# qiaozhijian/LPD-Net-Pytorch

Hardware: NVIDIA B200
Metric: LPD-Net eval embedding throughput (featnet=lpdnet, 4096 pts, k=20, NetVLAD K=64 D=1024 -> 256) (higher is better)
Workload: dtype f16

## Files before the change

### include/lpd_b200.h

```cpp
#ifndef LPD_B200_H
#define LPD_B200_H

#include <stddef.h>
#include <stdint.h>

#ifdef __cplusplus
extern "C" {
#endif

#define LPD_ABI_VERSION 2

typedef enum lpd_status {
    LPD_OK = 0,
    LPD_EINVAL = -1,
    LPD_EWORKSPACE = -2,
    LPD_ECUDA = -3,
    LPD_EUNSUPPORTED = -4
} lpd_status;

typedef enum lpd_act {
    LPD_ACT_NONE = 0,
    LPD_ACT_RELU = 1,
    LPD_ACT_LEAKY = 2,
    LPD_ACT_SIGMOID = 3,
    LPD_ACT_GATE = 4,
    LPD_ACT_ADD = 5
} lpd_act;

#define LPD_A_MK 0
#define LPD_A_KM 1
#define LPD_B_NK 0
#define LPD_B_KN 1

int lpd_abi_version(void);
const char* lpd_status_str(int status);
const char* lpd_last_cuda_error(void);
int lpd_device_info(int* sm_count, int* cc_major, int* cc_minor, size_t* smem_optin_bytes);

int lpd_bn_fold(const float* gamma, const float* beta, const float* mean, const float* var,
                const float* bias, float eps, int C, float* scale, float* shift, void* stream);

int lpd_transpose(const float* in, float* out, int batch, int rows, int cols, void* stream);

int lpd_knn(const float* x, int B, int N, int C, int k, void* idx, int idx_i64, void* stream);

size_t lpd_knn_workspace_bytes(int B, int N, int C, int k);
int lpd_knn_tc(const float* x, int B, int N, int C, int k, void* idx, int idx_i64,
               void* workspace, size_t workspace_bytes, void* stream);
int lpd_knn_tc_variant(int v);
size_t lpd_knn_tc_flags_offset(int B, int N, int C, int k);

size_t lpd_knn_xyz_workspace_bytes(int B, int N);
int lpd_knn_xyz(const float* x, int B, int N, int k, void* idx, int idx_i64, void* workspace, size_t workspace_bytes,
                void* stream);

int lpd_cell_order(const float* x, int B, int N, int32_t* perm, int32_t* inv, float* xyz_sorted,
                   void* workspace, size_t workspace_bytes, void* stream);

int lpd_cell_order_grid(const float* x, int B, int N, int32_t* perm, int32_t* inv, float* xyz_sorted,
                        void* workspace, size_t workspace_bytes, void* stream);
int lpd_knn_xyz_ordered(int B, int N, int k, void* idx, int idx_i64, void* workspace, size_t workspace_bytes, void* stream);

int lpd_gemm(const float* A, int a_layout, int lda, long long strideA,
             const float* B, int b_layout, int ldb, long long strideB,
             float* C, int ldc, long long strideC,
             int M, int N, int K, int batch,
             const float* scale, const float* shift, int act, float slope, const float* aux,
             void* stream);

int lpd_gemm_tf32(const float* A, int lda, const float* B, int ldb, float* C, int ldc,
                  int M, int N, int K, const float* scale, const float* shift, int act, float slope,
                  void* stream);
int lpd_gemm_tf32_ex(const float* A, int lda, const float* B, int ldb, float* C, int ldc,
                     int M, int N, int K, int batch, int accumulate, const float* scale, const float* shift, int act,
                     float slope, void* stream);

int lpd_gemm_tf32_tn(const float* A, int lda, const float* B, int ldb, float* C, int ldc, long long strideC,
                     int M, int N, int K, int batch, void* stream);

int lpd_gemm_f16(const void* A, int lda, const void* W, int ldw, void* C, int ldc, int out_half,
                 int M, int N, int K, const float* scale, const float* shift, int act, float slope, void* stream);
int lpd_gemm_f16_tn(const void* A, int lda, const void* B, int ldb, float* C, int ldc, long long strideC,
                    int M, int N, int K, int batch, void* stream);
int lpd_f32_to_f16(const float* x, long long ldx, void* y, long long ldy, long long rows, int cols, void* stream);
int lpd_split3_tf32(const float* x, long long n, float* out, int role, void* stream);
int lpd_transpose_split3(const float* v, int B, long long R, int Bp, float* out, void* stream);
int lpd_gemm_tf32_out16(const float* A, int lda, const float* B, int ldb, void* C, int ldc, int M, int N, int K,
                        const float* scale, const float* shift, int act, float slope, void* stream);
int lpd_softmax64_f16(float* a, long long M, void* a_h, void* stream);
int lpd_edge_gather_max_f16(const void* p, int ldp, const void* q, int ldq, const int32_t* idx, int B, int N, int k, int C,
                            int act, float slope, void* out, int ldo, void* stream);
int lpd_edgeconv_dg20_f16(const void* p, int ldp, const void* q, int ldq, const int32_t* idx, int B, int N,
                          const void* w2, const float* s2, const float* t2, int act, float slope,
                          void* x1, int ld1, void* x2, int ld2, void* stream);
int lpd_edgeconv_dg32_f16(const void* p, int ldp, const void* q, int ldq, const int32_t* idx, int B, int N,
                          const void* w2, const float* s2, const float* t2, int act, float slope,
                          void* x1, int ld1, void* x2, int ld2, void* stream);

int lpd_pointwise_mlp2(const float* x, int ldx, int D, long long M, const float* w1, const float* s1, const float* t1,
                       const float* w2, const float* s2, const float* t2, int act, float slope, float* out, int ldo,
                       void* stream);

int lpd_colmax(const float* x, int B, int N, int C, int ldx, float* out, void* stream);

int lpd_edge_gather_ext(const float* p, int ldp, const float* q, int ldq,
                        const int32_t* idx, int B, int N, int k, int C,
                        const float* scale, const float* shift, int act, float slope,
                        float* out, int ldo, void* stream);

int lpd_edgeconv_dg(const float* p, int ldp, const float* q, int ldq,
                    const int32_t* idx, int B, int N, int k, int C1, int C2,
                    const float* s1, const float* t1, const float* w2,
                    const float* s2, const float* t2, int act, float slope,
                    float* x1, int ld1, float* x2, int ld2, void* stream);

int lpd_edgeconv_dg_tf32(const float* p, int ldp, const float* q, int ldq,
                         const int32_t* idx, int B, int N, int k, int C1, int C2,
                         const float* s1, const float* t1, const float* w2,
                         const float* s2, const float* t2, int act, float slope,
                         float* x1, int ld1, float* x2, int ld2, void* stream);

int lpd_netvlad_assign(const float* x, int M, int D, const float* wc, const float* scale,
                       const float* shift, int K, float* a, void* stream);

int lpd_softmax64(float* a, long long M, void* stream);

int lpd_netvlad_finish(float* vlad, const float* a, const float* wc2, int B, int N, int D, int K,
                       float* asum_ws, void* stream);

int lpd_gemm_softmax64(const void* A, int a_f16, int lda, const void* W, int ldw, int M, int K, const float* scale,
                       const float* shift, float* a32, void* a16, float* apart, void* stream);

int lpd_netvlad_finish_parts(float* vlad, const float* apart, int nparts, const float* wc2, int B, int D, int K, void* stream);

int lpd_hidden_gate(const float* part, int splits, int B, int O, const float* s2, const float* t2, const float* wg,
                    const float* sg, const float* tg, float* out, void* stream);

int lpd_splitk_reduce(const float* part, int splits, int M, int N, const float* scale,
                      const float* shift, float* out, void* stream);

int lpd_quadruplet_loss(const float* q, const float* pos, const float* neg, const float* other,
                        int Bq, int P, int Nn, int D, float m1, float m2, int flags,
                        float* loss, float* gq, float* gpos, float* gneg, float* gother,
                        const float* grad_out, void* stream);

size_t lpd_retrieval_workspace_bytes(int Ndb, int Nq, int k);
int lpd_retrieval_topk(const float* db, int Ndb, const float* q, int Nq, int D, int k,
                       int idx_offset, int32_t* idx, double* dist,
                       void* workspace, size_t workspace_bytes, void* stream);

int lpd_topk_merge(const double* part_dist, const int32_t* part_idx, int lists, int Nq, int k,
                   int32_t* idx, double* dist, void* stream);

size_t lpd_retrieval_tc_workspace_bytes(int Ndb, int Nq, int D);
int lpd_retrieval_tc(const float* db, int Ndb, const float* q, int Nq, int D, int k,
                     const int32_t* seg_off, int S, int global_idx, int idx_offset,
                     int32_t* idx, double* dist, void* workspace, size_t workspace_bytes, void* stream);

int lpd_recall_count(const int32_t* idx, int S, int Nq, int k, const int32_t* q_run, int R, const int32_t* seg_run,
                     const int32_t* truth_off, const int32_t* truth_idx, const int32_t* seg_thresh,
                     const float* db, const int32_t* seg_off, const float* q, int D,
                     int32_t* hist, int32_t* n_eval, int32_t* n_onepct, float* sim, void* stream);


int lpd_bn_stats(const float* z, long long rows, int C, int ld, double* partial, int nparts, void* stream);
int lpd_bn_finalize(const double* partial, int nparts, double count, int C, const float* gamma, const float* beta,
                    float eps, float momentum, float* running_mean, float* running_var, float* bn_out, void* stream);
int lpd_colsum_finalize(const double* partial, int nparts, int n, float* out, void* stream);
int lpd_affine_act(const float* z, long long rows, int C, int ldz, const float* scale, const float* shift, int act,
                   float slope, const float* aux, int ldaux, float* out, int ldo, void* stream);
int lpd_bn_bwd_reduce(const float* dy, int lddy, const float* z, int ldz, long long rows, int C, const float* bn,
                      int act, float slope, const float* aux, int ldaux, double* partial, int nparts, void* stream);
int lpd_bn_bwd_apply(const float* dy, int lddy, const float* z, int ldz, long long rows, int C, const float* bn,
                     const float* S, double count, int act, float slope, const float* aux, int ldaux,
                     float* dz, int lddz, void* stream);

int lpd_edge_sel_stats(const float* p, int ldp, const float* q, int ldq, const int32_t* idx, int B, int N, int k, int C,
                       const float* gamma, float* zsel, int ldz, uint8_t* arg, double* partial, int nparts, void* stream);
int lpd_edge_materialize(const float* p, int ldp, const float* q, int ldq, const int32_t* idx, int B, int N, int k, int C,
                         const float* scale, const float* shift, int act, float slope, float* y, void* stream);
int lpd_edge_sel_dense(const float* z, long long M, int k, int C, const float* gamma, float* zsel, int ldz,
                       uint8_t* arg, void* stream);
int lpd_edge_dense_bwd_apply(const float* z, long long M, int k, int C, const float* bn, const float* S, double count,
                             int act, float slope, const float* dx, int lddx, const float* zsel, int ldzs,
                             const uint8_t* arg, float* dz, void* stream);
int lpd_edge_bwd_reduce(const float* p, int ldp, const float* q, int ldq, const int32_t* idx, int B, int N, int k, int C,
                        const float* bn, int act, float slope, const float* dx, int lddx, const uint8_t* arg,
                        const float* dy, double* partial, int nparts, void* stream);
int lpd_edge_bwd_apply(const float* p, int ldp, const float* q, int ldq, const int32_t* idx, int B, int N, int k, int C,
                       const float* bn, int act, float slope, const float* dx, int lddx, const uint8_t* arg,
                       const float* dy, const float* S, double count, float* dp, int lddp, float* dq, int lddq,
                       void* stream);

int lpd_edge_scatter_add(const float* dy, const int32_t* idx, int B, int N, int k, int C, float* dp, int lddp, void* stream);

int lpd_netvlad_finish_train(float* vlad, const float* a, const float* wc2, int B, int N, int D, int K,
                             float* asum, float* n1, float* n2, void* stream);
int lpd_netvlad_finish_bwd(float* dv, const float* v, const float* wc2, const float* asum, const float* n1,
                           const float* n2, int B, int D, int K, float* dasum, float* dwc2, void* stream);
int lpd_softmax64_bwd(float* da, const float* a, const float* dasum, long long M, int N, void* stream);

int lpd_colmax_arg(const float* x, int B, int N, int C, int ldx, float* out, int32_t* arg, void* stream);
int lpd_colmax_bwd(const float* dout, const int32_t* arg, int B, int N, int C, float* dx, int lddx, void* stream);

int lpd_adam(float* w, const float* g, float* m, float* v, long long n, float lr, float beta1, float beta2, float eps,
             float weight_decay, int step, float grad_scale, void* stream);
int lpd_axpy(float* y, int ldy, const float* x, int ldx, long long rows, int C, float alpha, void* stream);

#ifdef __cplusplus
}
#endif
#endif
```

### lpd-net-pytorch_b200/_lib.py

```python
from __future__ import annotations

import ctypes as C
import os
from pathlib import Path

_HERE = Path(__file__).resolve().parent
LIB_PATH = _HERE / "liblpd_b200.so"

LPD_OK = 0
ACT_NONE, ACT_RELU, ACT_LEAKY, ACT_SIGMOID, ACT_GATE, ACT_ADD = 0, 1, 2, 3, 4, 5
A_MK, A_KM = 0, 1
B_NK, B_KN = 0, 1
ABI_VERSION = 2

_vp, _i, _f, _ll, _sz, _d = C.c_void_p, C.c_int, C.c_float, C.c_longlong, C.c_size_t, C.c_double

SIGNATURES = {
    "lpd_abi_version": (_i, []),
    "lpd_status_str": (C.c_char_p, [_i]),
    "lpd_last_cuda_error": (C.c_char_p, []),
    "lpd_device_info": (_i, [C.POINTER(_i), C.POINTER(_i), C.POINTER(_i), C.POINTER(_sz)]),
    "lpd_bn_fold": (_i, [_vp, _vp, _vp, _vp, _vp, _f, _i, _vp, _vp, _vp]),
    "lpd_transpose": (_i, [_vp, _vp, _i, _i, _i, _vp]),
    "lpd_knn": (_i, [_vp, _i, _i, _i, _i, _vp, _i, _vp]),
    "lpd_knn_workspace_bytes": (_sz, [_i, _i, _i, _i]),
    "lpd_knn_tc": (_i, [_vp, _i, _i, _i, _i, _vp, _i, _vp, _sz, _vp]),
    "lpd_knn_tc_variant": (_i, [_i]),
    "lpd_knn_tc_flags_offset": (_sz, [_i, _i, _i, _i]),
    "lpd_knn_xyz_workspace_bytes": (_sz, [_i, _i]),
    "lpd_knn_xyz": (_i, [_vp, _i, _i, _i, _vp, _i, _vp, _sz, _vp]),
    "lpd_cell_order": (_i, [_vp, _i, _i, _vp, _vp, _vp, _vp, _sz, _vp]),
    "lpd_cell_order_grid": (_i, [_vp, _i, _i, _vp, _vp, _vp, _vp, _sz, _vp]),
    "lpd_knn_xyz_ordered": (_i, [_i, _i, _i, _vp, _i, _vp, _sz, _vp]),
    "lpd_gemm": (_i, [_vp, _i, _i, _ll, _vp, _i, _i, _ll, _vp, _i, _ll, _i, _i, _i, _i,
                      _vp, _vp, _i, _f, _vp, _vp]),
    "lpd_gemm_tf32": (_i, [_vp, _i, _vp, _i, _vp, _i, _i, _i, _i, _vp, _vp, _i, _f, _vp]),
    "lpd_gemm_tf32_ex": (_i, [_vp, _i, _vp, _i, _vp, _i, _i, _i, _i, _i, _i, _vp, _vp, _i, _f, _vp]),
    "lpd_gemm_tf32_tn": (_i, [_vp, _i, _vp, _i, _vp, _i, _ll, _i, _i, _i, _i, _vp]),
    "lpd_gemm_f16": (_i, [_vp, _i, _vp, _i, _vp, _i, _i, _i, _i, _i, _vp, _vp, _i, _f, _vp]),
    "lpd_gemm_f16_tn": (_i, [_vp, _i, _vp, _i, _vp, _i, _ll, _i, _i, _i, _i, _vp]),
    "lpd_f32_to_f16": (_i, [_vp, _ll, _vp, _ll, _ll, _i, _vp]),
    "lpd_split3_tf32": (_i, [_vp, _ll, _vp, _i, _vp]),
    "lpd_transpose_split3": (_i, [_vp, _i, _ll, _i, _vp, _vp]),
    "lpd_gemm_tf32_out16": (_i, [_vp, _i, _vp, _i, _vp, _i, _i, _i, _i, _vp, _vp, _i, _f, _vp]),
    "lpd_softmax64_f16": (_i, [_vp, _ll, _vp, _vp]),
    "lpd_edge_gather_max_f16": (_i, [_vp, _i, _vp, _i, _vp, _i, _i, _i, _i, _i, _f, _vp, _i, _vp]),
    "lpd_edgeconv_dg20_f16": (_i, [_vp, _i, _vp, _i, _vp, _i, _i, _vp, _vp, _vp, _i, _f, _vp, _i, _vp, _i, _vp]),
    "lpd_edgeconv_dg32_f16": (_i, [_vp, _i, _vp, _i, _vp, _i, _i, _vp, _vp, _vp, _i, _f, _vp, _i, _vp, _i, _vp]),
    "lpd_pointwise_mlp2": (_i, [_vp, _i, _i, _ll, _vp, _vp, _vp, _vp, _vp, _vp, _i, _f, _vp, _i, _vp]),
    "lpd_colmax": (_i, [_vp, _i, _i, _i, _i, _vp, _vp]),
    "lpd_edge_gather_ext": (_i, [_vp, _i, _vp, _i, _vp, _i, _i, _i, _i, _vp, _vp, _i, _f, _vp, _i, _vp]),
    "lpd_edgeconv_dg": (_i, [_vp, _i, _vp, _i, _vp, _i, _i, _i, _i, _i, _vp, _vp, _vp, _vp, _vp, _i, _f,
                             _vp, _i, _vp, _i, _vp]),
    "lpd_edgeconv_dg_tf32": (_i, [_vp, _i, _vp, _i, _vp, _i, _i, _i, _i, _i, _vp, _vp, _vp, _vp, _vp, _i, _f,
                                  _vp, _i, _vp, _i, _vp]),
    "lpd_netvlad_assign": (_i, [_vp, _i, _i, _vp, _vp, _vp, _i, _vp, _vp]),
    "lpd_softmax64": (_i, [_vp, _ll, _vp]),
    "lpd_netvlad_finish": (_i, [_vp, _vp, _vp, _i, _i, _i, _i, _vp, _vp]),
    "lpd_splitk_reduce": (_i, [_vp, _i, _i, _i, _vp, _vp, _vp, _vp]),
    "lpd_gemm_softmax64": (_i, [_vp, _i, _i, _vp, _i, _i, _i, _vp, _vp, _vp, _vp, _vp, _vp]),
    "lpd_netvlad_finish_parts": (_i, [_vp, _vp, _i, _vp, _i, _i, _i, _vp]),
    "lpd_hidden_gate": (_i, [_vp, _i, _i, _i, _vp, _vp, _vp, _vp, _vp, _vp, _vp]),
    "lpd_quadruplet_loss": (_i, [_vp, _vp, _vp, _vp, _i, _i, _i, _i, _f, _f, _i, _vp, _vp, _vp, _vp, _vp, _vp, _vp]),
    "lpd_retrieval_workspace_bytes": (_sz, [_i, _i, _i]),
    "lpd_retrieval_topk": (_i, [_vp, _i, _vp, _i, _i, _i, _i, _vp, _vp, _vp, _sz, _vp]),
    "lpd_topk_merge": (_i, [_vp, _vp, _i, _i, _i, _vp, _vp, _vp]),
    "lpd_retrieval_tc_workspace_bytes": (_sz, [_i, _i, _i]),
    "lpd_retrieval_tc": (_i, [_vp, _i, _vp, _i, _i, _i, _vp, _i, _i, _i, _vp, _vp, _vp, _sz, _vp]),
    "lpd_recall_count": (_i, [_vp, _i, _i, _i, _vp, _i, _vp, _vp, _vp, _vp, _vp, _vp, _vp, _i, _vp, _vp, _vp, _vp, _vp]),
    "lpd_bn_stats": (_i, [_vp, _ll, _i, _i, _vp, _i, _vp]),
    "lpd_bn_finalize": (_i, [_vp, _i, _d, _i, _vp, _vp, _f, _f, _vp, _vp, _vp, _vp]),
    "lpd_colsum_finalize": (_i, [_vp, _i, _i, _vp, _vp]),
    "lpd_affine_act": (_i, [_vp, _ll, _i, _i, _vp, _vp, _i, _f, _vp, _i, _vp, _i, _vp]),
    "lpd_bn_bwd_reduce": (_i, [_vp, _i, _vp, _i, _ll, _i, _vp, _i, _f, _vp, _i, _vp, _i, _vp]),
    "lpd_bn_bwd_apply": (_i, [_vp, _i, _vp, _i, _ll, _i, _vp, _vp, _d, _i, _f, _vp, _i, _vp, _i, _vp]),
    "lpd_edge_sel_stats": (_i, [_vp, _i, _vp, _i, _vp, _i, _i, _i, _i, _vp, _vp, _i, _vp, _vp, _i, _vp]),
    "lpd_edge_materialize": (_i, [_vp, _i, _vp, _i, _vp, _i, _i, _i, _i, _vp, _vp, _i, _f, _vp, _vp]),
    "lpd_edge_sel_dense": (_i, [_vp, _ll, _i, _i, _vp, _vp, _i, _vp, _vp]),
    "lpd_edge_dense_bwd_apply": (_i, [_vp, _ll, _i, _i, _vp, _vp, _d, _i, _f, _vp, _i, _vp, _i, _vp, _vp, _vp]),
    "lpd_edge_bwd_reduce": (_i, [_vp, _i, _vp, _i, _vp, _i, _i, _i, _i, _vp, _i, _f, _vp, _i, _vp, _vp, _vp, _i, _vp]),
    "lpd_edge_bwd_apply": (_i, [_vp, _i, _vp, _i, _vp, _i, _i, _i, _i, _vp, _i, _f, _vp, _i, _vp, _vp, _vp, _d,
                                _vp, _i, _vp, _i, _vp]),
    "lpd_edge_scatter_add": (_i, [_vp, _vp, _i, _i, _i, _i, _vp, _i, _vp]),
    "lpd_netvlad_finish_train": (_i, [_vp, _vp, _vp, _i, _i, _i, _i, _vp, _vp, _vp, _vp]),
    "lpd_netvlad_finish_bwd": (_i, [_vp, _vp, _vp, _vp, _vp, _vp, _i, _i, _i, _vp, _vp, _vp]),
    "lpd_softmax64_bwd": (_i, [_vp, _vp, _vp, _ll, _i, _vp]),
    "lpd_colmax_arg": (_i, [_vp, _i, _i, _i, _i, _vp, _vp, _vp]),
    "lpd_colmax_bwd": (_i, [_vp, _vp, _i, _i, _i, _vp, _i, _vp]),
    "lpd_adam": (_i, [_vp, _vp, _vp, _vp, _ll, _f, _f, _f, _f, _f, _i, _f, _vp]),
    "lpd_axpy": (_i, [_vp, _i, _vp, _i, _ll, _i, _f, _vp]),
}

_lib = None


class LpdError(RuntimeError):
    pass


def load() -> C.CDLL:
    global _lib
    if _lib is not None:
        return _lib
    path = Path(os.environ.get("LPD_B200_LIB", LIB_PATH))
    if not path.exists():
        raise LpdError(
            f"{path} not found: build it with `python -c 'import __graft_entry__ as g; g.build()'` "
            f"or `make -C {_HERE / 'csrc'}`; there is no CPU or torch fallback.")
    lib = C.CDLL(str(path))
    for name, (res, args) in SIGNATURES.items():
        fn = getattr(lib, name)
        fn.restype = res
        fn.argtypes = args
    if lib.lpd_abi_version() != ABI_VERSION:
        raise LpdError(f"ABI version mismatch: library {lib.lpd_abi_version()} != binding {ABI_VERSION}")
    _lib = lib
    return lib


def check(rc: int, what: str) -> None:
    if rc != LPD_OK:
        lib = load()
        msg = lib.lpd_status_str(rc).decode()
        detail = lib.lpd_last_cuda_error().decode()
        raise LpdError(f"{what} failed: {msg}" + (f" [{detail}]" if detail else ""))


def device_info() -> dict:
    lib = load()
    sm, maj, mnr, smem = _i(), _i(), _i(), _sz()
    check(lib.lpd_device_info(C.byref(sm), C.byref(maj), C.byref(mnr), C.byref(smem)), "lpd_device_info")
    return {"sm_count": sm.value, "cc": (maj.value, mnr.value), "smem_optin": smem.value}
```

### lpd-net-pytorch_b200/csrc/knn_tc.cu

```cuda
#include "tc_common.cuh"
#include "knn_select.cuh"

namespace lpd {

int knn_simt64_flagged(const float* x, int B, int N, int k, void* idx, int idx_i64, const int* flags, cudaStream_t st);

namespace tc {

constexpr int KT_Q = 128;
constexpr int KT_C = 64;
constexpr int KT_SCAN_WARPS = 8;
constexpr int KT_THREADS = 320;
constexpr int KT_STRIDE = 257;
constexpr int KT_BSTAGES = 3;
constexpr int KT_TSTAGES = 4;
constexpr int KT_XSLOTS = 8;

struct KnnTcParams {
    const float* xxpad;
    float* cand_v;
    int* cand_i;
    int B, N, Npad;
    int qtiles, ctiles;
};

__device__ __forceinline__ int ct_of(int s, int center, int ctiles) {
    const int d = (s + 1) >> 1;
    int ct = center + ((s & 1) ? d : -d);
    ct %= ctiles;
    return ct < 0 ? ct + ctiles : ct;
}

__device__ __forceinline__ float to_tf32(float v) {
    uint32_t r;
    asm("cvt.rna.tf32.f32 %0, %1;" : "=r"(r) : "f"(v));
    return __uint_as_float(r);
}

__global__ void __launch_bounds__(256)
knn_split_kernel(const float* __restrict__ x, int N, int Npad, float* __restrict__ x2, float* __restrict__ xxpad,
                 float* __restrict__ r2) {
    const int b = blockIdx.y;
    const int n = blockIdx.x * blockDim.x + threadIdx.x;
    if (n >= Npad) return;
    float v = INFINITY;
    if (n < N) {
        const float4* p = reinterpret_cast<const float4*>(x + ((size_t)b * N + n) * 64);
        float4* o = reinterpret_cast<float4*>(x2 + ((size_t)b * N + n) * 128);
        float acc = 0.f;
#pragma unroll
        for (int g = 0; g < 16; ++g) {
            const float4 t = __ldg(p + g);
            acc = __fmaf_rn(t.x, t.x, acc); acc = __fmaf_rn(t.y, t.y, acc);
            acc = __fmaf_rn(t.z, t.z, acc); acc = __fmaf_rn(t.w, t.w, acc);
            float4 hi, lo;
            hi.x = to_tf32(t.x); hi.y = to_tf32(t.y); hi.z = to_tf32(t.z); hi.w = to_tf32(t.w);
            lo.x = to_tf32(t.x - hi.x); lo.y = to_tf32(t.y - hi.y); lo.z = to_tf32(t.z - hi.z); lo.w = to_tf32(t.w - hi.w);
            o[g] = hi;
            o[16 + g] = lo;
        }
        v = acc;
        atomicMax(reinterpret_cast<int*>(r2 + b), __float_as_int(acc));
    }
    xxpad[(size_t)b * Npad + n] = v;
}

template <int GS, int QD>
struct KtSmem {
    static constexpr int L = 4 * GS;
    static constexpr uint32_t A_KB = KT_Q * 128;
    static constexpr uint32_t B_KB = KT_C * 128;
    static constexpr uint32_t A_BYTES = 4 * A_KB;
    static constexpr uint32_t B_BYTES = 4 * B_KB;
    static constexpr size_t off_b = A_BYTES;
    static constexpr size_t off_xs = off_b + KT_BSTAGES * B_BYTES;
    static constexpr size_t off_lv = off_xs + KT_XSLOTS * KT_C * 4;
    static constexpr size_t off_li = off_lv + (size_t)L * KT_STRIDE * 4;
    static constexpr size_t off_bar = (off_li + (size_t)L * KT_STRIDE * 4 + 7) / 8 * 8;
    static constexpr size_t total = off_bar + (2 + 2 * KT_BSTAGES + 2 * KT_TSTAGES) * 8 + 16;
    static_assert(total <= 227 * 1024, "knn_tc shared memory budget");
};

template <int GS, int QD>
__global__ void __launch_bounds__(KT_THREADS, 1)
knn_tc_kernel(const __grid_constant__ CUtensorMap tmap_a, const __grid_constant__ CUtensorMap tmap_b, KnnTcParams P) {
    using S = KtSmem<GS, QD>;
    constexpr int L = S::L;
    extern __shared__ __align__(1024) uint8_t smem[];
    if ((smem_u32(smem) & 1023u) != 0) __trap();
    uint8_t* a_s = smem;
    uint8_t* b_s = smem + S::off_b;
    float* xs = reinterpret_cast<float*>(smem + S::off_xs);
    float* lv = reinterpret_cast<float*>(smem + S::off_lv);
    int* li = reinterpret_cast<int*>(smem + S::off_li);
    uint64_t* afull = reinterpret_cast<uint64_t*>(smem + S::off_bar);
    uint64_t* aempty = afull + 1;
    uint64_t* bfull = aempty + 1;
    uint64_t* bempty = bfull + KT_BSTAGES;
    uint64_t* tfull = bempty + KT_BSTAGES;
    uint64_t* tempty = tfull + KT_TSTAGES;
    uint32_t* tmem_slot = reinterpret_cast<uint32_t*>(tempty + KT_TSTAGES);

    const int warp = threadIdx.x >> 5, lane = threadIdx.x & 31;
    const int items = P.B * P.qtiles;

    if (warp == 9) {
        if (lane == 0) {
            asm volatile("prefetch.tensormap [%0];" ::"l"(reinterpret_cast<uint64_t>(&tmap_a)) : "memory");
            asm volatile("prefetch.tensormap [%0];" ::"l"(reinterpret_cast<uint64_t>(&tmap_b)) : "memory");
            mbar_init(afull, 1); mbar_init(aempty, 1);
            for (int s = 0; s < KT_BSTAGES; ++s) { mbar_init(&bfull[s], 1); mbar_init(&bempty[s], 1); }
            for (int s = 0; s < KT_TSTAGES; ++s) { mbar_init(&tfull[s], 1); mbar_init(&tempty[s], KT_SCAN_WARPS); }
            asm volatile("fence.mbarrier_init.release.cluster;" ::: "memory");
        }
        __syncwarp();
        asm volatile("tcgen05.alloc.cta_group::1.sync.aligned.shared::cta.b32 [%0], 256;" ::"r"(smem_u32(tmem_slot)) : "memory");
        asm volatile("tcgen05.relinquish_alloc_permit.cta_group::1.sync.aligned;" ::: "memory");
    }
    tc_fence_before();
    __syncthreads();
    tc_fence_after();
    const uint32_t tmem_base = *tmem_slot;

    if (warp == 8) {
        if (lane == 0) {
            uint32_t tcount = 0, icount = 0;
            for (int item = blockIdx.x; item < items; item += gridDim.x, ++icount) {
                const int b = item / P.qtiles, q0 = (item % P.qtiles) * KT_Q;
                mbar_wait_sleep(aempty, (icount & 1) ^ 1);
                mbar_expect_tx(afull, S::A_BYTES);
#pragma unroll
                for (int kb = 0; kb < 4; ++kb) tma_load_2d(a_s + kb * S::A_KB, &tmap_a, afull, kb * 32, b * P.N + q0);
                for (int cs = 0; cs < P.ctiles; ++cs, ++tcount) {
                    const int ct = ct_of(cs, q0 / KT_C, P.ctiles);
                    const uint32_t s = tcount % KT_BSTAGES, ph = (tcount / KT_BSTAGES) & 1;
                    mbar_wait_sleep(&bempty[s], ph ^ 1);
                    mbar_expect_tx(&bfull[s], S::B_BYTES + KT_C * 4);
                    uint8_t* bs = b_s + s * S::B_BYTES;
#pragma unroll
                    for (int kb = 0; kb < 4; ++kb) tma_load_2d(bs + kb * S::B_KB, &tmap_b, &bfull[s], kb * 32, b * P.N + ct * KT_C);
                    asm volatile("cp.async.bulk.shared::cluster.global.mbarrier::complete_tx::bytes [%0], [%1], %2, [%3];"
                                 ::"r"(smem_u32(xs + (tcount % KT_XSLOTS) * KT_C)), "l"(P.xxpad + (size_t)b * P.Npad + ct * KT_C),
                                   "r"(KT_C * 4), "r"(smem_u32(&bfull[s])) : "memory");
                }
            }
        }
    } else if (warp == 9) {
        if (lane == 0) {
            constexpr uint32_t idesc = make_idesc(KT_Q, KT_C);
            const uint32_t a_addr = smem_u32(a_s);
            uint32_t tcount = 0, icount = 0;
            for (int item = blockIdx.x; item < items; item += gridDim.x, ++icount) {
                mbar_wait_sleep(afull, icount & 1);
                for (int ct = 0; ct < P.ctiles; ++ct, ++tcount) {
                    const uint32_t s = tcount % KT_BSTAGES, ph = (tcount / KT_BSTAGES) & 1;
                    const uint32_t ts = tcount % KT_TSTAGES, tph = (tcount / KT_TSTAGES) & 1;
                    mbar_wait_sleep(&tempty[ts], tph ^ 1);
                    mbar_wait_sleep(&bfull[s], ph);
                    tc_fence_after();
                    const uint32_t b_addr = smem_u32(b_s + s * S::B_BYTES);
                    const uint32_t d = tmem_base + ts * KT_C;
                    uint32_t acc = 0;
#pragma unroll
                    for (int term = 0; term < 3; ++term) {
                        const int akb = (term == 1) ? 2 : 0, bkb = (term == 0) ? 2 : 0;
#pragma unroll
                        for (int kb = 0; kb < 2; ++kb) {
                            const uint64_t da = make_smem_desc(a_addr + (akb + kb) * S::A_KB);
                            const uint64_t db = make_smem_desc(b_addr + (bkb + kb) * S::B_KB);
#pragma unroll
                            for (int ks = 0; ks < 4; ++ks) {
                                tc_mma_tf32(d, da + (uint64_t)(ks * 2), db + (uint64_t)(ks * 2), idesc, acc);
                                acc = 1;
                            }
                        }
                    }
                    tc_commit(&bempty[s]);
                    tc_commit(&tfull[ts]);
                }
                tc_commit(aempty);
            }
        }
    } else {
        const int quad = warp & 3, half = warp >> 2;
        const int own = half * KT_Q + quad * 32 + lane;
        RowSelect<GS, false, KT_STRIDE> sel;
        uint32_t tcount = 0;
        for (int item = blockIdx.x; item < items; item += gridDim.x) {
            const int b = item / P.qtiles, q0 = (item % P.qtiles) * KT_Q;
            sel.reset();
            for (int cs = 0; cs < P.ctiles; ++cs, ++tcount) {
                const int ct = ct_of(cs, q0 / KT_C, P.ctiles);
                const uint32_t ts = tcount % KT_TSTAGES, tph = (tcount / KT_TSTAGES) & 1;
                mbar_wait(&tfull[ts], tph);
                tc_fence_after();
                const float* xsj = xs + (tcount % KT_XSLOTS) * KT_C + half * 32;
                uint32_t r[32];
                tc_ld32(tmem_base + ((uint32_t)(quad * 32) << 16) + ts * KT_C + half * 32, r);
                tc_fence_before();
                __syncwarp();
                if (lane == 0) mbar_arrive(&tempty[ts]);
                const int jbase = ct * KT_C + half * 32;
#pragma unroll
                for (int sub = 0; sub < 32 / QD; ++sub) {
                    float a[QD];
                    float m4[4] = {-INFINITY, -INFINITY, -INFINITY, -INFINITY};
#pragma unroll
                    for (int j = 0; j < QD; j += 4) {
                        const float4 xx = *reinterpret_cast<const float4*>(xsj + sub * QD + j);
                        a[j + 0] = fmaf(2.f, __uint_as_float(r[sub * QD + j + 0]), -xx.x);
                        a[j + 1] = fmaf(2.f, __uint_as_float(r[sub * QD + j + 1]), -xx.y);
                        a[j + 2] = fmaf(2.f, __uint_as_float(r[sub * QD + j + 2]), -xx.z);
                        a[j + 3] = fmaf(2.f, __uint_as_float(r[sub * QD + j + 3]), -xx.w);
                        m4[0] = fmaxf(m4[0], a[j]); m4[1] = fmaxf(m4[1], a[j + 1]);
                        m4[2] = fmaxf(m4[2], a[j + 2]); m4[3] = fmaxf(m4[3], a[j + 3]);
                    }
                    const float mx = fmaxf(fmaxf(m4[0], m4[1]), fmaxf(m4[2], m4[3]));
                    uint32_t mask = 0;
                    if (mx > sel.tau) {
#pragma unroll
                        for (int j = 0; j < QD; ++j) mask |= (a[j] > sel.tau) ? (1u << j) : 0u;
                    }
                    while (__any_sync(kFull, mask != 0)) {
                        if (mask) {
                            const int j = __ffs(mask) - 1;
                            mask &= mask - 1;
                            float t[QD];
#pragma unroll
                            for (int q = 0; q < QD; ++q) t[q] = a[q];
#pragma unroll
                            for (int w = QD / 2, bit = 0; w >= 1; w >>= 1, ++bit) {
                                const bool hi = (j >> bit) & 1;
#pragma unroll
                                for (int q = 0; q < w; ++q) t[q] = hi ? t[2 * q + 1] : t[2 * q];
                            }
                            sel.insert(lv, li, own, t[0], jbase + sub * QD + j);
                        }
                    }
                }
            }
            __syncwarp();
            for (int rl = 0; rl < 32; ++rl) {
                const int qrow = q0 + quad * 32 + rl;
                const int nfill = __shfl_sync(kFull, sel.filled, rl);
                if (qrow >= P.N) break;
                const size_t o = (((size_t)b * P.N + qrow) * 2 + half) * L;
                const int src = half * KT_Q + quad * 32 + rl;
                for (int s = lane; s < L; s += 32) {
                    const bool valid = s < nfill;
                    P.cand_v[o + s] = valid ? lv[s * KT_STRIDE + src] : -INFINITY;
                    P.cand_i[o + s] = valid ? li[s * KT_STRIDE + src] : INT_MAX;
                }
            }
            __syncwarp();
        }
    }
    tc_fence_before();
    __syncthreads();
    if (warp == 9) {
        tc_fence_after();
        asm volatile("tcgen05.dealloc.cta_group::1.sync.aligned.b32 %0, 256;" ::"r"(tmem_base) : "memory");
    }
}

__global__ void __launch_bounds__(256)
knn_refine_kernel(const float* __restrict__ x, const float* __restrict__ xxpad, const float* __restrict__ r2,
                  const float* __restrict__ cand_v, const int* __restrict__ cand_i, int Lh, int B, int N, int Npad, int k,
                  void* __restrict__ idx_out, int idx_i64, int* __restrict__ flags) {
    constexpr int E = 2;
    const int lane = threadIdx.x & 31;
    const long long grow = (long long)blockIdx.x * 8 + (threadIdx.x >> 5);
    if (grow >= (long long)B * N) return;
    const int b = (int)(grow / N), qi = (int)(grow % N);
    const int L = 2 * Lh;
    float av[E]; int id[E];
    float tmin[2] = {INFINITY, INFINITY};
    bool hfull[2] = {true, true};
#pragma unroll
    for (int e = 0; e < E; ++e) {
        const int s = e * 32 + lane;
        av[e] = -INFINITY; id[e] = INT_MAX;
        if (s < L) {
            av[e] = cand_v[grow * L + s];
            id[e] = cand_i[grow * L + s];
            const int h = s >= Lh;
            if (id[e] == INT_MAX || id[e] >= N) {
                id[e] = INT_MAX;
                if (h) hfull[1] = false; else hfull[0] = false;
            } else {
                if (h) tmin[1] = fminf(tmin[1], av[e]); else tmin[0] = fminf(tmin[0], av[e]);
            }
        }
    }
#pragma unroll
    for (int o = 16; o > 0; o >>= 1) {
        tmin[0] = fminf(tmin[0], __shfl_xor_sync(kFull, tmin[0], o));
        tmin[1] = fminf(tmin[1], __shfl_xor_sync(kFull, tmin[1], o));
    }
    const bool full0 = __all_sync(kFull, hfull[0]), full1 = __all_sync(kFull, hfull[1]);
    const float tau = fmaxf(full0 ? tmin[0] : -INFINITY, full1 ? tmin[1] : -INFINITY);
    const float xxi = __ldg(xxpad + (size_t)b * Npad + qi);
    const float rmax2 = __ldg(r2 + b);
    const float eps = 6.103515625e-5f * sqrtf(xxi) * sqrtf(rmax2) + 9.5367431640625e-7f * (xxi + rmax2);
    warp_sort_desc<E>(av, id, lane);
    const float a_k = __shfl_sync(kFull, av[0], k - 1);
    const float cut = a_k - 2.f * eps;
    const float4* xi = reinterpret_cast<const float4*>(x + ((size_t)b * N + qi) * 64);
    float pd[E];
#pragma unroll
    for (int e = 0; e < E; ++e) {
        pd[e] = -INFINITY;
        const bool keep = (id[e] != INT_MAX) && (av[e] >= cut);
        if (!keep) id[e] = INT_MAX;
        if (__any_sync(kFull, keep)) {
            if (keep) {
                const float4* xj = reinterpret_cast<const float4*>(x + ((size_t)b * N + id[e]) * 64);
                float dot = 0.f;
#pragma unroll
                for (int g = 0; g < 16; ++g) {
                    const float4 u = __ldg(xi + g), w = __ldg(xj + g);
                    dot = __fmaf_rn(u.x, w.x, dot); dot = __fmaf_rn(u.y, w.y, dot);
                    dot = __fmaf_rn(u.z, w.z, dot); dot = __fmaf_rn(u.w, w.w, dot);
                }
                const float xxj = __ldg(xxpad + (size_t)b * Npad + id[e]);
                const float t = -2.0f * dot;
                pd[e] = __fsub_rn(__fsub_rn(-xxj, t), xxi);
            }
        }
    }
    warp_sort_desc<E>(pd, id, lane);
    const float pd_k = __shfl_sync(kFull, pd[0], k - 1);
    const bool ok = (tau == -INFINITY) || (tau + eps < pd_k + xxi);
    const size_t o = (size_t)grow * k;
#pragma unroll
    for (int e = 0; e < E; ++e) {
        const int g = e * 32 + lane;
        if (g < k) {
            if (idx_i64) reinterpret_cast<long long*>(idx_out)[o + g] = id[e];
            else reinterpret_cast<int*>(idx_out)[o + g] = id[e];
        }
    }
    if (!ok && lane == 0) flags[(size_t)b * ((N + 63) / 64) + qi / 64] = 1;
}

template <int GS, int QD>
static int knn_tc_launch(const CUtensorMap& ta, const CUtensorMap& tb, const KnnTcParams& P, cudaStream_t st) {
    const size_t smem = KtSmem<GS, QD>::total;
    LPD_CUDA_CHECK(allow_smem(knn_tc_kernel<GS, QD>, smem));
    int dev = 0, sms = 0;
    LPD_CUDA_CHECK(cudaGetDevice(&dev));
    LPD_CUDA_CHECK(cudaDeviceGetAttribute(&sms, cudaDevAttrMultiProcessorCount, dev));
    const int items = P.B * P.qtiles;
    knn_tc_kernel<GS, QD><<<items < sms ? items : sms, KT_THREADS, smem, st>>>(ta, tb, P);
    LPD_LAUNCH_CHECK();
    return LPD_OK;
}

static inline size_t align_up(size_t v, size_t a) { return (v + a - 1) / a * a; }

struct KnnWs {
    size_t off_xx, off_r2, off_flags, off_x2, off_cv, off_ci, total;
    int npad, L;
    KnnWs(int B, int N, int k) {
        npad = (N + 127) / 128 * 128;
        L = k <= 24 ? 48 : 64;
        size_t o = 0;
        off_xx = o; o = align_up(o + (size_t)B * npad * 4, 256);
        off_r2 = o; o += (size_t)B * 4;
        off_flags = o; o = align_up(o + (size_t)B * ((N + 63) / 64) * 4, 256);
        off_x2 = o; o = align_up(o + (size_t)B * N * 128 * 4, 256);
        off_cv = o; o = align_up(o + (size_t)B * N * L * 4, 256);
        off_ci = o; o = align_up(o + (size_t)B * N * L * 4, 256);
        total = o;
    }
};

}
}

namespace lpd { namespace tc {
size_t knn2_workspace_bytes(int B, int N, int k);
size_t knn2_flags_offset(int B, int N, int k);
int knn2_run(const float* x, int B, int N, int k, void* idx, int idx_i64, void* workspace, size_t workspace_bytes, int mt,
             cudaStream_t st);
static int g_knn_variant = 1;
}}

extern "C" int lpd_knn_tc_variant(int v) {
    const int prev = lpd::tc::g_knn_variant;
    if (v >= 0 && v <= 3) lpd::tc::g_knn_variant = v;
    return prev;
}

extern "C" size_t lpd_knn_workspace_bytes(int B, int N, int C, int k) {
    if (B < 1 || N < 1 || C != 64 || k < 1 || k > 32) return 0;
    const size_t a = lpd::tc::KnnWs(B, N, k).total, b = lpd::tc::knn2_workspace_bytes(B, N, k);
    return a > b ? a : b;
}

extern "C" size_t lpd_knn_tc_flags_offset(int B, int N, int C, int k) {
    if (B < 1 || N < 1 || C != 64 || k < 1 || k > 32) return 0;
    return lpd::tc::g_knn_variant == 0 ? lpd::tc::KnnWs(B, N, k).off_flags : lpd::tc::knn2_flags_offset(B, N, k);
}

extern "C" int lpd_knn_tc(const float* x, int B, int N, int C, int k, void* idx, int idx_i64,
                          void* workspace, size_t workspace_bytes, void* stream) {
    using namespace lpd;
    LPD_REQUIRE(x && idx && workspace);
    LPD_REQUIRE(B >= 1 && B <= 65535 && N >= 1 && C == 64 && k >= 1 && k <= 32 && k <= N);
    LPD_REQUIRE((long long)B * N < (1ll << 31) / 128);
    LPD_REQUIRE(((uintptr_t)x & 15) == 0 && ((uintptr_t)workspace & 255) == 0);
    const tc::KnnWs W(B, N, k);
    if (workspace_bytes < lpd_knn_workspace_bytes(B, N, C, k)) return LPD_EWORKSPACE;
    int dev = 0, major = 0;
    LPD_CUDA_CHECK(cudaGetDevice(&dev));
    LPD_CUDA_CHECK(cudaDeviceGetAttribute(&major, cudaDevAttrComputeCapabilityMajor, dev));
    if (major != 10) return LPD_EUNSUPPORTED;
    cudaStream_t st = as_stream(stream);
    if (tc::g_knn_variant != 0) return tc::knn2_run(x, B, N, k, idx, idx_i64, workspace, workspace_bytes, tc::g_knn_variant, st);
    uint8_t* ws = reinterpret_cast<uint8_t*>(workspace);
    float* xxpad = reinterpret_cast<float*>(ws + W.off_xx);
    float* r2 = reinterpret_cast<float*>(ws + W.off_r2);
    int* flags = reinterpret_cast<int*>(ws + W.off_flags);
    float* x2 = reinterpret_cast<float*>(ws + W.off_x2);
    const int ftiles = (N + 63) / 64;
    LPD_CUDA_CHECK(cudaMemsetAsync(r2, 0, (size_t)B * sizeof(float), st));
    LPD_CUDA_CHECK(cudaMemsetAsync(flags, 0, (size_t)B * ftiles * sizeof(int), st));
    tc::knn_split_kernel<<<dim3(ceil_div(W.npad, 256), B), 256, 0, st>>>(x, N, W.npad, x2, xxpad, r2);
    LPD_LAUNCH_CHECK();
    CUtensorMap ta, tb;
    int rc = tc::make_tmap(&ta, x2, (long long)B * N, 128, 128, tc::KT_Q);
    if (rc != LPD_OK) return rc;
    rc = tc::make_tmap(&tb, x2, (long long)B * N, 128, 128, tc::KT_C);
    if (rc != LPD_OK) return rc;
    tc::KnnTcParams P;
    P.xxpad = xxpad;
    P.cand_v = reinterpret_cast<float*>(ws + W.off_cv);
    P.cand_i = reinterpret_cast<int*>(ws + W.off_ci);
    P.B = B; P.N = N; P.Npad = W.npad; P.qtiles = ceil_div(N, tc::KT_Q); P.ctiles = ceil_div(N, tc::KT_C);
    rc = (W.L == 48) ? tc::knn_tc_launch<6, 16>(ta, tb, P, st) : tc::knn_tc_launch<8, 16>(ta, tb, P, st);
    if (rc != LPD_OK) return rc;
    const unsigned rblocks = (unsigned)(((long long)B * N + 7) / 8);
    tc::knn_refine_kernel<<<rblocks, 256, 0, st>>>(x, xxpad, r2, P.cand_v, P.cand_i, W.L / 2, B, N, W.npad, k, idx, idx_i64, flags);
    LPD_LAUNCH_CHECK();
    return knn_simt64_flagged(x, B, N, k, idx, idx_i64, flags, st);
}
```

### lpd-net-pytorch_b200/csrc/knn_tc2.cu

```cuda
#include "tc_common.cuh"
#include <cuda_fp16.h>
#include <limits.h>
#include <stdlib.h>

namespace lpd {

int knn_simt64_list(const float* x, int B, int N, int k, void* idx, int idx_i64, const int* list, cudaStream_t st);

namespace tc {

constexpr int K2_C = 128;
constexpr int K2_BSTAGES = 4;
constexpr int K2_TCOLS = 512;
constexpr int K2_XSLOTS = 12;
constexpr int K2_TBL = 128;

struct Knn2Params {
    const float* nrmpad;
    const float* snpad;
    const uint4* xh;
    const uint4* ext;
    const float* xxpad;
    const float* r2;
    const float* r2c;
    const float* sc;
    int* cnt;
    int* cand;
    int B, N, Npad, k;
    int qtiles, ctiles;
};

__device__ __forceinline__ void tc_mma_f16(uint32_t tmem_d, uint64_t desc_a, uint64_t desc_b, uint32_t idesc, uint32_t accumulate) {
    asm volatile(
        "{\n\t.reg .pred p;\n\t"
        "setp.ne.b32 p, %4, 0;\n\t"
        "tcgen05.mma.cta_group::1.kind::f16 [%0], %1, %2, %3, p;\n\t}"
        ::"r"(tmem_d), "l"(desc_a), "l"(desc_b), "r"(idesc), "r"(accumulate)
        : "memory");
}
__device__ __forceinline__ void tc_mma_f16_p(uint32_t tmem_d, uint64_t desc_a, uint64_t desc_b, uint32_t idesc, uint32_t accumulate,
                                             uint32_t leader) {
    asm volatile(
        "{\n\t.reg .pred p, q;\n\t"
        "setp.ne.b32 p, %4, 0;\n\t"
        "elect.sync _|q, 0xffffffff;\n\t"
        "@q tcgen05.mma.cta_group::1.kind::f16 [%0], %1, %2, %3, p;\n\t}"
        ::"r"(tmem_d), "l"(desc_a), "l"(desc_b), "r"(idesc), "r"(accumulate), "r"(leader)
        : "memory");
}
__device__ __forceinline__ void tc_commit_p(uint64_t* bar, uint32_t leader) {
    asm volatile(
        "{\n\t.reg .pred q;\n\t"
        "elect.sync _|q, 0xffffffff;\n\t"
        "@q tcgen05.commit.cta_group::1.mbarrier::arrive::one.shared::cluster.b64 [%0];\n\t}"
        ::"r"(smem_u32(bar)), "r"(leader) : "memory");
}
__device__ __forceinline__ void tma_load_2d_p(void* smem_dst, const CUtensorMap* tmap, uint64_t* bar, int c0, int c1, uint32_t leader) {
    asm volatile(
        "{\n\t.reg .pred q;\n\t"
        "elect.sync _|q, 0xffffffff;\n\t"
        "@q cp.async.bulk.tensor.2d.shared::cluster.global.mbarrier::complete_tx::bytes [%0], [%1, {%3, %4}], [%2];\n\t}"
        ::"r"(smem_u32(smem_dst)), "l"(reinterpret_cast<uint64_t>(tmap)), "r"(smem_u32(bar)), "r"(c0), "r"(c1), "r"(leader)
        : "memory");
}
__device__ __forceinline__ void bulk_load_p(void* smem_dst, const void* gsrc, uint32_t bytes, uint64_t* bar, uint32_t leader) {
    asm volatile(
        "{\n\t.reg .pred q;\n\t"
        "elect.sync _|q, 0xffffffff;\n\t"
        "@q cp.async.bulk.shared::cluster.global.mbarrier::complete_tx::bytes [%0], [%1], %2, [%3];\n\t}"
        ::"r"(smem_u32(smem_dst)), "l"(gsrc), "r"(bytes), "r"(smem_u32(bar)), "r"(leader) : "memory");
}
__device__ __forceinline__ void mbar_expect_tx_p(uint64_t* bar, uint32_t bytes, uint32_t leader) {
    asm volatile(
        "{\n\t.reg .pred q;\n\t"
        "elect.sync _|q, 0xffffffff;\n\t"
        "@q mbarrier.arrive.expect_tx.shared::cta.b64 _, [%0], %1;\n\t}"
        ::"r"(smem_u32(bar)), "r"(bytes), "r"(leader) : "memory");
}
__device__ __forceinline__ void tc_mma_f16_ts(uint32_t tmem_d, uint32_t tmem_a, uint64_t desc_b, uint32_t idesc, uint32_t accumulate) {
    asm volatile(
        "{\n\t.reg .pred p, q;\n\t"
        "setp.ne.b32 p, %4, 0;\n\t"
        "elect.sync _|q, 0xffffffff;\n\t"
        "@q tcgen05.mma.cta_group::1.kind::f16 [%0], [%1], %2, %3, p;\n\t}"
        ::"r"(tmem_d), "r"(tmem_a), "l"(desc_b), "r"(idesc), "r"(accumulate)
        : "memory");
}
__device__ __forceinline__ void tc_st4(uint32_t taddr, const uint4& v) {
    asm volatile("tcgen05.st.sync.aligned.32x32b.x4.b32 [%0], {%1, %2, %3, %4};"
                 ::"r"(taddr), "r"(v.x), "r"(v.y), "r"(v.z), "r"(v.w) : "memory");
}
__host__ __device__ constexpr uint32_t make_idesc_f16(int M, int N) {
    return (1u << 4) | ((uint32_t)(N >> 3) << 17) | ((uint32_t)(M >> 4) << 24);
}
__device__ __forceinline__ void named_bar(int id, int nthreads) {
    asm volatile("bar.sync %0, %1;" ::"r"(id), "r"(nthreads) : "memory");
}

__host__ __device__ __forceinline__ void block_perm(int t, int& a, int& b) {
    const uint32_t v = (uint32_t)(t + 1) * 2654435761u;
    a = (int)((v >> 8) & 63u) | 1;
    b = (int)((v >> 20) & 63u);
}
__host__ __device__ __forceinline__ int inv_mod64(int a) {
    return (a * (2 - a * a)) & 63;
}

constexpr int K2_CSPLIT = 8;
__global__ void __launch_bounds__(256)
knn2_center_kernel(const float* __restrict__ x, int N, float* __restrict__ part) {
    __shared__ float4 red[3][256];
    __shared__ int sbad;
    const int b = blockIdx.y, sp = blockIdx.x, t = threadIdx.x, cg = t & 15, rl = t >> 4;
    const int chunk = (N + K2_CSPLIT - 1) / K2_CSPLIT;
    const int n0 = sp * chunk, n1 = min(N, n0 + chunk);
    const float4* xb = reinterpret_cast<const float4*>(x + (size_t)b * N * 64);
    if (t == 0) sbad = 0;
    float4 s = make_float4(0.f, 0.f, 0.f, 0.f);
    float4 lo = make_float4(INFINITY, INFINITY, INFINITY, INFINITY), hi = make_float4(-INFINITY, -INFINITY, -INFINITY, -INFINITY);
    bool bad = false;
    for (int n = n0 + rl; n < n1; n += 16) {
        const float4 v = __ldg(xb + (size_t)n * 16 + cg);
        s.x += v.x; s.y += v.y; s.z += v.z; s.w += v.w;
        lo.x = fminf(lo.x, v.x); lo.y = fminf(lo.y, v.y); lo.z = fminf(lo.z, v.z); lo.w = fminf(lo.w, v.w);
        hi.x = fmaxf(hi.x, v.x); hi.y = fmaxf(hi.y, v.y); hi.z = fmaxf(hi.z, v.z); hi.w = fmaxf(hi.w, v.w);
        bad |= !(fabsf(v.x) <= 3.0e38f) || !(fabsf(v.y) <= 3.0e38f) || !(fabsf(v.z) <= 3.0e38f) || !(fabsf(v.w) <= 3.0e38f);
    }
    red[0][t] = s; red[1][t] = lo; red[2][t] = hi;
    __syncthreads();
    if (bad) sbad = 1;
    for (int o = 128; o >= 16; o >>= 1) {
        if (t < o) {
            const float4 a0 = red[0][t], c0 = red[0][t + o], a1 = red[1][t], c1 = red[1][t + o], a2 = red[2][t], c2 = red[2][t + o];
            red[0][t] = make_float4(a0.x + c0.x, a0.y + c0.y, a0.z + c0.z, a0.w + c0.w);
            red[1][t] = make_float4(fminf(a1.x, c1.x), fminf(a1.y, c1.y), fminf(a1.z, c1.z), fminf(a1.w, c1.w));
            red[2][t] = make_float4(fmaxf(a2.x, c2.x), fmaxf(a2.y, c2.y), fmaxf(a2.z, c2.z), fmaxf(a2.w, c2.w));
        }
        __syncthreads();
    }
    float* o = part + ((size_t)b * K2_CSPLIT + sp) * 196;
    if (t < 16) {
        reinterpret_cast<float4*>(o)[t] = red[0][t];
        reinterpret_cast<float4*>(o + 64)[t] = red[1][t];
        reinterpret_cast<float4*>(o + 128)[t] = red[2][t];
    }
    if (t == 0) o[192] = sbad ? 1.f : 0.f;
}

__device__ __forceinline__ void knn2_fold_center(const float* __restrict__ part, int b, int N, float* mus, float* ssc, float* red) {
    const int t = threadIdx.x;
    if (t < 64) {
        const float* pb = part + (size_t)b * K2_CSPLIT * 196;
        float s = 0.f, lo = INFINITY, hi = -INFINITY, bad = 0.f;
#pragma unroll
        for (int sp = 0; sp < K2_CSPLIT; ++sp) {
            s += pb[sp * 196 + t];
            lo = fminf(lo, pb[sp * 196 + 64 + t]);
            hi = fmaxf(hi, pb[sp * 196 + 128 + t]);
            bad += pb[sp * 196 + 192];
        }
        const float m = s * (1.f / (float)N);
        mus[t] = m;
        float g = fmaxf(hi - m, m - lo);
        if (bad != 0.f || !(g <= 3.0e38f)) g = INFINITY;
        red[t] = g;
    }
    __syncthreads();
    if (t == 0) {
        float g = 0.f;
        for (int c = 0; c < 64; ++c) g = fmaxf(g, red[c]);
        float sigma = 1.f, c2 = 2.f;
        if (g > 0.f) {
            int e;
            frexpf(g, &e);
            const int se = 8 - e;
            if (!(g <= 3.0e38f) || se > 60 || se < -60) {
                sigma = 1.f; c2 = __int_as_float(0x7fc00000);
            } else {
                sigma = ldexpf(1.f, se);
                c2 = ldexpf(2.f, -2 * se);
            }
        }
        ssc[0] = sigma; ssc[1] = c2;
    }
    __syncthreads();
}

constexpr int K2_PREP_XS = 68;
constexpr int K2_PREP_HS = 9;
constexpr size_t K2_PREP_SMEM = 256 * K2_PREP_XS * 4 + 256 * K2_PREP_HS * 16;
__global__ void __launch_bounds__(256)
knn2_prep_kernel(const float* __restrict__ x, const float* __restrict__ part, float* __restrict__ sc, int N, int Npad,
                 __half* __restrict__ xh, uint4* __restrict__ ext, float* __restrict__ xxpad, float* __restrict__ nrmpad,
                 float* __restrict__ snpad, float* __restrict__ r2, float* __restrict__ r2c) {
    __shared__ __align__(16) float mus_f[64];
    __shared__ float ssc[2], sred[64];
    extern __shared__ __align__(16) uint8_t prep_sm[];
    float* xs = reinterpret_cast<float*>(prep_sm);
    uint4* hs = reinterpret_cast<uint4*>(prep_sm + 256 * K2_PREP_XS * 4);
    const int b = blockIdx.y;
    const int n0 = blockIdx.x * 256;
    {
        const float4* src = reinterpret_cast<const float4*>(x + ((size_t)b * N + n0) * 64);
        const int rows = min(256, N - n0);
#pragma unroll 4
        for (int i = threadIdx.x; i < rows * 16; i += 256)
            *reinterpret_cast<float4*>(xs + (i >> 4) * K2_PREP_XS + (i & 15) * 4) = __ldg(src + i);
    }
    knn2_fold_center(part, b, N, mus_f, ssc, sred);
    const float4* mus = reinterpret_cast<const float4*>(mus_f);
    const float sigma = ssc[0];
    if (blockIdx.x == 0 && threadIdx.x == 0) { sc[2 * b] = sigma; sc[2 * b + 1] = ssc[1]; }
    const int n = n0 + threadIdx.x;
    float vxx = INFINITY, vn = INFINITY;
    int np = n;
    if ((n | 63) < N) {
        int a, bb;
        block_perm(n >> 6, a, bb);
        np = (n & ~63) | (((n & 63) * a + bb) & 63);
    }
    if (n < N) {
        const float4* p = reinterpret_cast<const float4*>(xs + threadIdx.x * K2_PREP_XS);
        uint4* o = hs + (np - n0) * K2_PREP_HS;
        float acc = 0.f, accc = 0.f;
#pragma unroll
        for (int g = 0; g < 8; ++g) {
            const float4 t0 = p[2 * g], t1 = p[2 * g + 1];
            acc = __fmaf_rn(t0.x, t0.x, acc); acc = __fmaf_rn(t0.y, t0.y, acc);
            acc = __fmaf_rn(t0.z, t0.z, acc); acc = __fmaf_rn(t0.w, t0.w, acc);
            acc = __fmaf_rn(t1.x, t1.x, acc); acc = __fmaf_rn(t1.y, t1.y, acc);
            acc = __fmaf_rn(t1.z, t1.z, acc); acc = __fmaf_rn(t1.w, t1.w, acc);
            const float4 m0 = mus[2 * g], m1 = mus[2 * g + 1];
            float c[8] = {t0.x - m0.x, t0.y - m0.y, t0.z - m0.z, t0.w - m0.w, t1.x - m1.x, t1.y - m1.y, t1.z - m1.z, t1.w - m1.w};
#pragma unroll
            for (int q = 0; q < 8; ++q) accc = __fmaf_rn(c[q], c[q], accc);
            uint32_t pk[4];
#pragma unroll
            for (int q = 0; q < 4; ++q) {
                const __half2 h = __floats2half2_rn(c[2 * q] * sigma, c[2 * q + 1] * sigma);
                pk[q] = *reinterpret_cast<const uint32_t*>(&h);
            }
            o[g] = make_uint4(pk[0], pk[1], pk[2], pk[3]);
        }
        vxx = acc; vn = accc;
        atomicMax(reinterpret_cast<int*>(r2 + b), __float_as_int(acc));
        atomicMax(reinterpret_cast<int*>(r2c + b), __float_as_int(accc));
    }
    __syncthreads();
    {
        uint4* dst = reinterpret_cast<uint4*>(xh + ((size_t)b * N + n0) * 64);
        const int rows = min(256, N - n0);
#pragma unroll 4
        for (int i = threadIdx.x; i < rows * 8; i += 256) dst[i] = hs[(i >> 3) * K2_PREP_HS + (i & 7)];
    }
    {
        float b1 = 0.f, b2 = 0.f, b3 = 0.f, b4 = -60000.f;
        if (n < N) {
            const float V = 0.5f * (sigma * sigma) * vn;
            b1 = __half2float(__float2half_rn(V * 0.015625f));
            const float r1 = __fmaf_rn(-b1, 64.f, V);
            b2 = __half2float(__float2half_rn(r1 * 32.f));
            const float rr = __fmaf_rn(-b2, 0.03125f, r1);
            b3 = __half2float(__float2half_rn(rr * 16384.f));
            b4 = 0.f;
        }
        const __half2 h01 = __floats2half2_rn(-b1, -b2), h23 = __floats2half2_rn(-b3, b4);
        const int r = np & 63;
        uint4* e = ext + ((size_t)b * (Npad >> 6) + (np >> 6)) * 128 + (r >> 3) * 16 + (r & 7);
        e[0] = make_uint4(*reinterpret_cast<const uint32_t*>(&h01), *reinterpret_cast<const uint32_t*>(&h23), 0u, 0u);
        e[8] = make_uint4(0u, 0u, 0u, 0u);
    }
    xxpad[(size_t)b * Npad + n] = vxx;
    nrmpad[(size_t)b * Npad + np] = vn;
    snpad[(size_t)b * Npad + np] = n < N ? sqrtf(vn) : 0.f;
}

__device__ __forceinline__ void cex_desc(float& a, float& b) {
    const float hi = fmaxf(a, b), lo = fminf(a, b);
    a = hi; b = lo;
}
__device__ __forceinline__ void bitonic_merge32_desc(float (&v)[32]) {
#pragma unroll
    for (int stride = 16; stride > 0; stride >>= 1) {
#pragma unroll
        for (int i = 0; i < 32; ++i)
            if ((i & stride) == 0) cex_desc(v[i], v[i | stride]);
    }
}
__device__ __forceinline__ void bitonic_sort32_desc(float (&v)[32]) {
#pragma unroll
    for (int size = 2; size <= 32; size <<= 1) {
#pragma unroll
        for (int stride = size >> 1; stride > 0; stride >>= 1) {
#pragma unroll
            for (int i = 0; i < 32; ++i) {
                if ((i & stride) == 0) {
                    const bool desc = ((i & size) == 0) || (size == 32);
                    if (desc) cex_desc(v[i], v[i | stride]); else cex_desc(v[i | stride], v[i]);
                }
            }
        }
    }
}

__device__ __forceinline__ uint64_t make_smem_desc_ext(uint32_t smem_addr) {
    uint64_t d = 0;
    d |= (uint64_t)((smem_addr & 0x3FFFF) >> 4);
    d |= (uint64_t)(128 >> 4) << 16;
    d |= (uint64_t)(256 >> 4) << 32;
    d |= (uint64_t)1 << 46;
    return d;
}
__device__ __forceinline__ void tc_ld32x2(uint32_t taddr, uint32_t (&a)[32], uint32_t (&b)[32]) {
#define LPD_LD32(R, ADDR)                                                                                               \
    asm volatile(                                                                                                       \
        "tcgen05.ld.sync.aligned.32x32b.x32.b32 "                                                                       \
        "{%0, %1, %2, %3, %4, %5, %6, %7, %8, %9, %10, %11, %12, %13, %14, %15, "                                       \
        "%16, %17, %18, %19, %20, %21, %22, %23, %24, %25, %26, %27, %28, %29, %30, %31}, [%32];"                       \
        : "=r"(R[0]), "=r"(R[1]), "=r"(R[2]), "=r"(R[3]), "=r"(R[4]), "=r"(R[5]), "=r"(R[6]), "=r"(R[7]),              \
          "=r"(R[8]), "=r"(R[9]), "=r"(R[10]), "=r"(R[11]), "=r"(R[12]), "=r"(R[13]), "=r"(R[14]), "=r"(R[15]),        \
          "=r"(R[16]), "=r"(R[17]), "=r"(R[18]), "=r"(R[19]), "=r"(R[20]), "=r"(R[21]), "=r"(R[22]), "=r"(R[23]),      \
          "=r"(R[24]), "=r"(R[25]), "=r"(R[26]), "=r"(R[27]), "=r"(R[28]), "=r"(R[29]), "=r"(R[30]), "=r"(R[31])       \
        : "r"(ADDR))
    LPD_LD32(a, taddr);
    LPD_LD32(b, taddr + 64);
#undef LPD_LD32
    asm volatile("tcgen05.wait::ld.sync.aligned;" ::: "memory");
}
__device__ __forceinline__ int fkey(float v) {
    const int b = __float_as_int(v);
    return b ^ ((b >> 31) & 0x7fffffff);
}
__device__ __forceinline__ float fmax3(float a, float b, float c) {
    float r;
    asm("max.f32 %0, %1, %2, %3;" : "=f"(r) : "f"(a), "f"(b), "f"(c));
    return r;
}

template <int MT, bool TS = false>
struct K2Smem {
    static constexpr int SCAN_THREADS = 256 * MT;
    static constexpr int TSTAGES = TS ? 3 : K2_TCOLS / (K2_C * MT);
    static constexpr int EXS = SCAN_THREADS + 1;
    static constexpr uint32_t A_TILE = 128 * 128;
    static constexpr uint32_t A_BYTES = MT * A_TILE;
    static constexpr uint32_t B_BYTES = K2_C * 128;
    static constexpr uint32_t BX_BYTES = K2_C * 32;
    static constexpr size_t off_b = TS ? 0 : 2 * A_BYTES;
    static constexpr size_t off_bx = off_b + K2_BSTAGES * B_BYTES;
    static constexpr size_t off_ax = off_bx + K2_BSTAGES * BX_BYTES;
    static constexpr size_t off_xs = off_ax + 128 * 32;
    static constexpr size_t off_ex = off_xs + K2_XSLOTS * K2_C * 4;
    static constexpr size_t off_tbl = off_ex + (size_t)32 * EXS * 4;
    static constexpr size_t off_bar = (off_tbl + (size_t)8 * MT * K2_TBL * 4 + 7) / 8 * 8;
    static constexpr size_t total = off_bar + (4 + 2 * K2_BSTAGES + 2 * TSTAGES) * 8 + 16;
    static_assert(total <= 227 * 1024, "knn2 shared memory budget");
};

template <int MT, int CAP, bool TIGHT, bool TS>
__global__ void __launch_bounds__(256 * MT + 64, 1)
knn2_tc_kernel(const __grid_constant__ CUtensorMap tmap_a, const __grid_constant__ CUtensorMap tmap_b, Knn2Params P) {
    static_assert(!TS || MT == 1, "TS mode: one 128-row query tile per item");
    using S = K2Smem<MT, TS>;
    constexpr int SCAN_WARPS = 8 * MT;
    constexpr uint32_t ACOL = 384;
    constexpr int TCOLS = K2_C * MT;
    constexpr int K2_TSTAGES = S::TSTAGES;
    extern __shared__ __align__(1024) uint8_t smem[];
    if ((smem_u32(smem) & 1023u) != 0) __trap();
    uint8_t* a_s = smem;
    uint8_t* b_s = smem + S::off_b;
    uint8_t* bx_s = smem + S::off_bx;
    uint8_t* ax_s = smem + S::off_ax;
    float* xs = reinterpret_cast<float*>(smem + S::off_xs);
    float* ex = reinterpret_cast<float*>(smem + S::off_ex);
    int* tbl = reinterpret_cast<int*>(smem + S::off_tbl);
    uint64_t* afull = reinterpret_cast<uint64_t*>(smem + S::off_bar);
    uint64_t* aempty = afull + 2;
    uint64_t* bfull = aempty + 2;
    uint64_t* bempty = bfull + K2_BSTAGES;
    uint64_t* tfull = bempty + K2_BSTAGES;
    uint64_t* tempty = tfull + K2_TSTAGES;
    uint32_t* tmem_slot = reinterpret_cast<uint32_t*>(tempty + K2_TSTAGES);

    const int warp = threadIdx.x >> 5, lane = threadIdx.x & 31;
    const int items = P.B * P.qtiles;
    const int nstages = 2 * P.ctiles;
    const int full_blocks = P.N >> 6;

    if (threadIdx.x < 128) {
        const int r = threadIdx.x;
        const __half2 h01 = __floats2half2_rn(64.f, 0.03125f), h23 = __floats2half2_rn(6.103515625e-05f, 32768.f);
        uint4* e = reinterpret_cast<uint4*>(ax_s) + (r >> 3) * 16 + (r & 7);
        e[0] = make_uint4(*reinterpret_cast<const uint32_t*>(&h01), *reinterpret_cast<const uint32_t*>(&h23), 0u, 0u);
        e[8] = make_uint4(0u, 0u, 0u, 0u);
        asm volatile("fence.proxy.async.shared::cta;" ::: "memory");
    }
    if (warp == SCAN_WARPS + 1) {
        if (lane == 0) {
            asm volatile("prefetch.tensormap [%0];" ::"l"(reinterpret_cast<uint64_t>(&tmap_a)) : "memory");
            asm volatile("prefetch.tensormap [%0];" ::"l"(reinterpret_cast<uint64_t>(&tmap_b)) : "memory");
            for (int s = 0; s < 2; ++s) { mbar_init(&afull[s], TS ? SCAN_WARPS : 1); mbar_init(&aempty[s], 1); }
            for (int s = 0; s < K2_BSTAGES; ++s) { mbar_init(&bfull[s], 1); mbar_init(&bempty[s], 1); }
            for (int s = 0; s < K2_TSTAGES; ++s) { mbar_init(&tfull[s], 1); mbar_init(&tempty[s], SCAN_WARPS); }
            asm volatile("fence.mbarrier_init.release.cluster;" ::: "memory");
        }
        __syncwarp();
        asm volatile("tcgen05.alloc.cta_group::1.sync.aligned.shared::cta.b32 [%0], %1;" ::"r"(smem_u32(tmem_slot)), "r"(TS ? 512 : TCOLS * K2_TSTAGES) : "memory");
        asm volatile("tcgen05.relinquish_alloc_permit.cta_group::1.sync.aligned;" ::: "memory");
    }
    tc_fence_before();
    __syncthreads();
    tc_fence_after();
    const uint32_t tmem_base = *tmem_slot;

    if (warp == SCAN_WARPS) {
        {
            const uint32_t leader = lane == 0;
            uint32_t tcount = 0, icount = 0;
            for (int item = blockIdx.x; item < items; item += gridDim.x, ++icount) {
                const int b = item / P.qtiles, q0 = (item % P.qtiles) * (128 * MT);
                const uint32_t ab = icount & 1, aph = (icount >> 1) & 1;
                if (!TS) {
                    mbar_wait_sleep(&aempty[ab], aph ^ 1);
                    mbar_expect_tx_p(&afull[ab], S::A_BYTES, leader);
#pragma unroll
                    for (int mt = 0; mt < MT; ++mt)
                        tma_load_2d_p(a_s + ab * S::A_BYTES + mt * S::A_TILE, &tmap_a, &afull[ab], 0, b * P.N + q0 + mt * 128, leader);
                }
                const uint4* extb = P.ext + (size_t)b * (P.Npad >> 6) * 128;
                const float* snb = P.snpad + (size_t)b * P.Npad;
                uint32_t s = tcount % K2_BSTAGES, ph = (tcount / K2_BSTAGES) & 1, xsl = tcount % K2_XSLOTS;
                for (int cs = 0; cs < nstages; ++cs, ++tcount) {
                    const int ct = cs >= P.ctiles ? cs - P.ctiles : cs;
                    mbar_wait_sleep(&bempty[s], ph ^ 1);
                    mbar_expect_tx_p(&bfull[s], S::B_BYTES + S::BX_BYTES + (TIGHT ? K2_C * 4 : 0), leader);
                    tma_load_2d_p(b_s + s * S::B_BYTES, &tmap_b, &bfull[s], 0, b * P.N + ct * K2_C, leader);
                    bulk_load_p(bx_s + s * S::BX_BYTES, extb + (size_t)ct * 256, S::BX_BYTES, &bfull[s], leader);
                    if (TIGHT) bulk_load_p(xs + xsl * K2_C, snb + ct * K2_C, K2_C * 4, &bfull[s], leader);
                    if (++s == K2_BSTAGES) { s = 0; ph ^= 1; }
                    xsl = (xsl + 1) % K2_XSLOTS;
                }
            }
        }
    } else if (warp == SCAN_WARPS + 1) {
        {
            constexpr uint32_t idesc = make_idesc_f16(128, K2_C);
            const uint32_t leader = lane == 0;
            const uint64_t dax = make_smem_desc_ext(smem_u32(ax_s));
            uint32_t tcount = 0, icount = 0;
            for (int item = blockIdx.x; item < items; item += gridDim.x, ++icount) {
                const uint32_t ab = icount & 1, aph = (icount >> 1) & 1;
                mbar_wait_sleep(&afull[ab], aph);
                if (TS) tc_fence_after();
                const uint64_t da0 = make_smem_desc(smem_u32(a_s + ab * S::A_BYTES));
                const uint32_t ta0 = tmem_base + ACOL + ab * 64;
                uint32_t s = tcount % K2_BSTAGES, ph = (tcount / K2_BSTAGES) & 1;
                uint32_t ts = tcount % K2_TSTAGES, tph = (tcount / K2_TSTAGES) & 1;
                for (int cs = 0; cs < nstages; ++cs, ++tcount) {
                    mbar_wait(&tempty[ts], tph ^ 1);
                    mbar_wait(&bfull[s], ph);
                    tc_fence_after();
                    const uint64_t db = make_smem_desc(smem_u32(b_s + s * S::B_BYTES));
                    const uint64_t dbx = make_smem_desc_ext(smem_u32(bx_s + s * S::BX_BYTES));
                    if (TS) {
                        const uint32_t d = tmem_base + ts * TCOLS;
#pragma unroll
                        for (int ks = 0; ks < 4; ++ks) tc_mma_f16_ts(d, ta0 + ks * 8, db + (uint64_t)(ks * 2), idesc, ks ? 1u : 0u);
                        tc_mma_f16_ts(d, ta0 + 32, dbx, idesc, 1u);
                    } else {
#pragma unroll
                        for (int ks = 0; ks < 5; ++ks) {
#pragma unroll
                            for (int mt = 0; mt < MT; ++mt) {
                                const uint64_t da = da0 + (uint64_t)(mt * (S::A_TILE >> 4));
                                const uint32_t d = tmem_base + ts * TCOLS + mt * K2_C;
                                if (ks < 4) tc_mma_f16_p(d, da + (uint64_t)(ks * 2), db + (uint64_t)(ks * 2), idesc, ks ? 1u : 0u, leader);
                                else tc_mma_f16_p(d, dax, dbx, idesc, 1u, leader);
                            }
                        }
                    }
                    tc_commit_p(&bempty[s], leader);
                    tc_commit_p(&tfull[ts], leader);
                    if (++s == K2_BSTAGES) { s = 0; ph ^= 1; }
                    if (++ts == K2_TSTAGES) { ts = 0; tph ^= 1; }
                }
                tc_commit_p(&aempty[ab], leader);
            }
        }
    } else {
        const int quad = warp & 3, half = (warp >> 2) & 1, mt = warp >> 3;
        const int own = mt * 256 + half * 128 + quad * 32 + lane;
        const int partner = own ^ 128;
        const uint32_t tm_lane = ((uint32_t)(quad * 32) << 16) + mt * K2_C + half * 32;
        uint32_t tcount = 0, icount = 0;
        uint4 aw[5];
        auto load_a = [&](int it2) {
            const int b2 = it2 / P.qtiles, q02 = (it2 % P.qtiles) * 128;
            const long long grow = (long long)b2 * P.N + q02 + quad * 32 + lane;
            const bool inb = grow < (long long)P.B * P.N;
            const uint4* src = P.xh + grow * 8;
            const uint4 zero = make_uint4(0u, 0u, 0u, 0u);
            if (half == 0) {
#pragma unroll
                for (int i = 0; i < 5; ++i) aw[i] = inb ? __ldg(src + i) : zero;
            } else {
#pragma unroll
                for (int i = 0; i < 3; ++i) aw[i] = inb ? __ldg(src + 5 + i) : zero;
                const __half2 h01 = __floats2half2_rn(64.f, 0.03125f), h23 = __floats2half2_rn(6.103515625e-05f, 32768.f);
                aw[3] = make_uint4(*reinterpret_cast<const uint32_t*>(&h01), *reinterpret_cast<const uint32_t*>(&h23), 0u, 0u);
                aw[4] = zero;
            }
        };
        auto store_a = [&](uint32_t n) {
            const uint32_t buf = n & 1, use = n >> 1;
            mbar_wait(&aempty[buf], (use & 1) ^ 1);
            const uint32_t ta = tmem_base + ((uint32_t)(quad * 32) << 16) + ACOL + buf * 64 + half * 20;
#pragma unroll
            for (int i = 0; i < 5; ++i) tc_st4(ta + 4 * i, aw[i]);
            asm volatile("tcgen05.wait::st.sync.aligned;" ::: "memory");
            tc_fence_before();
            __syncwarp();
            if (lane == 0) mbar_arrive(&afull[buf]);
        };
        if (TS && blockIdx.x < items) { load_a(blockIdx.x); store_a(0); }
        for (int item = blockIdx.x; item < items; item += gridDim.x, ++icount) {
            const int b = item / P.qtiles, q0 = (item % P.qtiles) * (128 * MT);
            const bool have_next = TS && item + (int)gridDim.x < items;
            if (have_next) load_a(item + gridDim.x);
            const int srow = q0 + mt * 128 + quad * 32 + lane;
            int row = srow;
            if ((srow >> 6) < full_blocks) {
                int a, bb;
                block_perm(srow >> 6, a, bb);
                row = (srow & ~63) | ((((srow & 63) - bb) * inv_mod64(a)) & 63);
            }
            const bool live = srow < P.N;
            const float inv_cb = 1.f / __ldg(P.sc + 2 * b + 1);
            float ni = 0.f, cni = 0.f, gself = 0.f;
            if (live) {
                const float ni2 = __ldg(P.nrmpad + (size_t)b * P.Npad + srow);
                ni = sqrtf(ni2); cni = 2.5e-3f * ni * inv_cb;
                gself = ni2 * inv_cb;
            }
            const bool use_tbl = P.ctiles <= K2_TBL;
            int* wtbl = tbl + warp * K2_TBL;
            const float ub_extra = TIGHT ? cni * sqrtf(__ldg(P.r2c + b)) : 0.f;
            float m[32];
#pragma unroll
            for (int j = 0; j < 32; ++j) m[j] = -INFINITY;
            for (int cs = 0; cs < P.ctiles; ++cs, ++tcount) {
                const uint32_t ts = tcount % K2_TSTAGES, tph = (tcount / K2_TSTAGES) & 1;
                mbar_wait(&tfull[ts], tph);
                tc_fence_after();
                uint32_t r0[32], r1[32];
                tc_ld32x2(tmem_base + tm_lane + ts * TCOLS, r0, r1);
                tc_fence_before();
                __syncwarp();
                if (lane == 0) mbar_arrive(&tempty[ts]);
                float tm = -INFINITY;
                if (TIGHT) {
                    const float* xsj = xs + (tcount % K2_XSLOTS) * K2_C + half * 32;
#pragma unroll
                    for (int j = 0; j < 32; j += 4) {
                        const float4 s0 = *reinterpret_cast<const float4*>(xsj + j), s1 = *reinterpret_cast<const float4*>(xsj + 64 + j);
                        m[j + 0] = fmax3(m[j + 0], fmaf(-cni, s0.x, __uint_as_float(r0[j + 0])), fmaf(-cni, s1.x, __uint_as_float(r1[j + 0])));
                        m[j + 1] = fmax3(m[j + 1], fmaf(-cni, s0.y, __uint_as_float(r0[j + 1])), fmaf(-cni, s1.y, __uint_as_float(r1[j + 1])));
                        m[j + 2] = fmax3(m[j + 2], fmaf(-cni, s0.z, __uint_as_float(r0[j + 2])), fmaf(-cni, s1.z, __uint_as_float(r1[j + 2])));
                        m[j + 3] = fmax3(m[j + 3], fmaf(-cni, s0.w, __uint_as_float(r0[j + 3])), fmaf(-cni, s1.w, __uint_as_float(r1[j + 3])));
                    }
                } else {
#pragma unroll
                    for (int j = 0; j < 32; ++j) m[j] = fmax3(m[j], __uint_as_float(r0[j]), __uint_as_float(r1[j]));
                }
                if (use_tbl) {
#pragma unroll
                    for (int j = 0; j < 32; ++j) tm = fmax3(tm, __uint_as_float(r0[j]), __uint_as_float(r1[j]));
                    const float D = live ? gself - (tm + ub_extra) : INFINITY;
                    const int dk = __reduce_min_sync(kFull, fkey(D));
                    if (lane == 0) wtbl[cs] = dk;
                }
            }
            bitonic_sort32_desc(m);
#pragma unroll
            for (int j = 0; j < 32; ++j) ex[j * S::EXS + own] = m[j];
            named_bar(1, S::SCAN_THREADS);
#pragma unroll
            for (int j = 0; j < 32; ++j) m[j] = fmaxf(m[j], ex[(31 - j) * S::EXS + partner]);
            named_bar(2, S::SCAN_THREADS);
            bitonic_merge32_desc(m);
            float tau0 = m[0];
#pragma unroll
            for (int j = 1; j < 32; ++j) tau0 = (j == P.k - 1) ? m[j] : tau0;
            float thr = INFINITY;
            if (live) {
                const float xxi = __ldg(P.xxpad + (size_t)b * P.Npad + row);
                const float r2 = __ldg(P.r2 + b), r2c = __ldg(P.r2c + b), sigma = __ldg(P.sc + 2 * b);
                const float rc = sqrtf(r2c);
                float eps = (1.9e-6f / sigma) * (ni + rc) + 7.62939453125e-6f * (xxi + r2) + 3.814697265625e-6f * r2c;
                if (!TIGHT) eps += 2.5e-3f * ni * rc;
                thr = fmaxf(tau0 - 2.f * eps * inv_cb, -1.0e9f);
                if (!(eps * inv_cb < INFINITY)) thr = __int_as_float(0x7fc00000);
            }
            if (have_next) store_a(icount + 1);
            const int dthr = __reduce_max_sync(kFull, fkey(live ? gself - thr : -INFINITY));
            int cnt = 0;
            int* mine = P.cand + (((size_t)b * P.N + (live ? row : 0)) * 2 + half) * CAP;
            for (int cs = 0; cs < P.ctiles; ++cs, ++tcount) {
                const uint32_t ts = tcount % K2_TSTAGES, tph = (tcount / K2_TSTAGES) & 1;
                mbar_wait(&tfull[ts], tph);
                if (use_tbl && wtbl[cs] > dthr) {
                    __syncwarp();
                    if (lane == 0) mbar_arrive(&tempty[ts]);
                    continue;
                }
                tc_fence_after();
                uint32_t r0[32], r1[32];
                tc_ld32x2(tmem_base + tm_lane + ts * TCOLS, r0, r1);
                tc_fence_before();
                __syncwarp();
                if (lane == 0) mbar_arrive(&tempty[ts]);
                float u0[32], u1[32];
                if (TIGHT) {
                    const float* xsj = xs + (tcount % K2_XSLOTS) * K2_C + half * 32;
#pragma unroll
                    for (int j = 0; j < 32; j += 4) {
                        const float4 s0 = *reinterpret_cast<const float4*>(xsj + j), s1 = *reinterpret_cast<const float4*>(xsj + 64 + j);
                        u0[j + 0] = fmaf(cni, s0.x, __uint_as_float(r0[j + 0])); u1[j + 0] = fmaf(cni, s1.x, __uint_as_float(r1[j + 0]));
                        u0[j + 1] = fmaf(cni, s0.y, __uint_as_float(r0[j + 1])); u1[j + 1] = fmaf(cni, s1.y, __uint_as_float(r1[j + 1]));
                        u0[j + 2] = fmaf(cni, s0.z, __uint_as_float(r0[j + 2])); u1[j + 2] = fmaf(cni, s1.z, __uint_as_float(r1[j + 2]));
                        u0[j + 3] = fmaf(cni, s0.w, __uint_as_float(r0[j + 3])); u1[j + 3] = fmaf(cni, s1.w, __uint_as_float(r1[j + 3]));
                    }
                } else {
#pragma unroll
                    for (int j = 0; j < 32; ++j) { u0[j] = __uint_as_float(r0[j]); u1[j] = __uint_as_float(r1[j]); }
                }
                float mx = -INFINITY;
#pragma unroll
                for (int j = 0; j < 32; ++j) mx = fmax3(mx, u0[j], u1[j]);
                if (__any_sync(kFull, mx >= thr)) {
                    uint32_t mask0 = 0, mask1 = 0;
#pragma unroll
                    for (int j = 0; j < 32; ++j) {
                        mask0 |= (u0[j] >= thr) ? (1u << j) : 0u;
                        mask1 |= (u1[j] >= thr) ? (1u << j) : 0u;
                    }
                    int pa0 = 1, pb0 = 0, pa1 = 1, pb1 = 0;
                    if (2 * cs < full_blocks) { block_perm(2 * cs, pa0, pb0); pa0 = inv_mod64(pa0); }
                    if (2 * cs + 1 < full_blocks) { block_perm(2 * cs + 1, pa1, pb1); pa1 = inv_mod64(pa1); }
                    const int jbase = cs * K2_C, pos0 = half * 32;
                    while (mask0) {
                        const int j = __ffs(mask0) - 1;
                        mask0 &= mask0 - 1;
                        if (cnt < CAP) mine[cnt] = jbase + (((pos0 + j - pb0) * pa0) & 63);
                        ++cnt;
                    }
                    while (mask1) {
                        const int j = __ffs(mask1) - 1;
                        mask1 &= mask1 - 1;
                        if (cnt < CAP) mine[cnt] = jbase + 64 + (((pos0 + j - pb1) * pa1) & 63);
                        ++cnt;
                    }
                }
            }
            if (live) P.cnt[((size_t)b * P.N + row) * 2 + half] = cnt;
        }
    }
    tc_fence_before();
    __syncthreads();
    if (warp == SCAN_WARPS + 1) {
        tc_fence_after();
        asm volatile("tcgen05.dealloc.cta_group::1.sync.aligned.b32 %0, %1;" ::"r"(tmem_base), "r"(TS ? 512 : TCOLS * K2_TSTAGES) : "memory");
    }
}

__device__ __forceinline__ void knn2_flag_tile(int* __restrict__ flags, int* __restrict__ list, int tile) {
    if (atomicExch(flags + tile, 1) == 0) list[1 + atomicAdd(list, 1)] = tile;
}
constexpr int RF_STRIDE = 36;
constexpr int RF_WARPS = 8;
template <int CAP>
struct RefineSmem {
    static constexpr int KEYS = 2 * CAP + 2;
    static constexpr size_t rows = (size_t)RF_WARPS * 32 * RF_STRIDE * 4;
    static constexpr size_t off_xi = rows;
    static constexpr size_t off_key = off_xi + (size_t)RF_WARPS * 64 * 4;
    static constexpr size_t off_id = off_key + (size_t)RF_WARPS * KEYS * 8;
    static constexpr size_t total = off_id + (size_t)RF_WARPS * 2 * CAP * 4;
};

template <int CAP>
__global__ void __launch_bounds__(RF_WARPS * 32)
knn2_refine_kernel(const float* __restrict__ x, const float* __restrict__ xxpad, const int* __restrict__ cnt,
                   const int* __restrict__ cand, int B, int N, int Npad, int k, void* __restrict__ idx_out, int idx_i64,
                   int* __restrict__ flags, int* __restrict__ list) {
    using S = RefineSmem<CAP>;
    extern __shared__ __align__(16) uint8_t rsm[];
    const int lane = threadIdx.x & 31, w = threadIdx.x >> 5;
    float* s_rows = reinterpret_cast<float*>(rsm) + (size_t)w * 32 * RF_STRIDE;
    float* s_xi = reinterpret_cast<float*>(rsm + S::off_xi) + w * 64;
    unsigned long long* s_key = reinterpret_cast<unsigned long long*>(rsm + S::off_key) + w * S::KEYS;
    int* s_id = reinterpret_cast<int*>(rsm + S::off_id) + w * 2 * CAP;
    const long long grow = (long long)blockIdx.x * RF_WARPS + w;
    if (grow >= (long long)B * N) return;
    const int b = (int)(grow / N), qi = (int)(grow % N);
    const int c0 = __ldg(cnt + grow * 2), c1 = __ldg(cnt + grow * 2 + 1);
    const int total = c0 + c1;
    if (c0 > CAP || c1 > CAP || total < k) {
        if (lane == 0) knn2_flag_tile(flags, list, b * ((N + 63) / 64) + qi / 64);
        return;
    }
    const float* xb = x + (size_t)b * N * 64;
    reinterpret_cast<float2*>(s_xi)[lane] = __ldg(reinterpret_cast<const float2*>(xb + (size_t)qi * 64) + lane);
    const float xxi = __ldg(xxpad + (size_t)b * Npad + qi);
    const int* l0 = cand + (size_t)grow * 2 * CAP;
    for (int s = lane; s < total; s += 32) s_id[s] = s < c0 ? __ldg(l0 + s) : __ldg(l0 + CAP + (s - c0));
    if (lane < 2) s_key[total + lane] = 0ull;
    __syncwarp();
    const int qw = lane >> 3, ql = lane & 7;
    for (int base = 0; base < total; base += 32) {
        const int nc = min(32, total - base);
        const int myid = lane < nc ? s_id[base + lane] : 0;
        float dot = 0.f;
#pragma unroll
        for (int ph = 0; ph < 2; ++ph) {
            __syncwarp();
            for (int c = qw; c < nc; c += 4) {
                const int j = s_id[base + c];
                const float4 v = __ldg(reinterpret_cast<const float4*>(xb + (size_t)j * 64 + ph * 32) + ql);
                *reinterpret_cast<float4*>(s_rows + c * RF_STRIDE + ql * 4) = v;
            }
            __syncwarp();
            if (lane < nc) {
                const float4* rj = reinterpret_cast<const float4*>(s_rows + lane * RF_STRIDE);
#pragma unroll
                for (int g = 0; g < 8; ++g) {
                    const float4 u = reinterpret_cast<const float4*>(s_xi)[ph * 8 + g], v = rj[g];
                    dot = __fmaf_rn(u.x, v.x, dot); dot = __fmaf_rn(u.y, v.y, dot);
                    dot = __fmaf_rn(u.z, v.z, dot); dot = __fmaf_rn(u.w, v.w, dot);
                }
            }
        }
        if (lane < nc) {
            const float xxj = __ldg(xxpad + (size_t)b * Npad + myid);
            const float t = -2.0f * dot;
            const float pd = __fadd_rn(__fsub_rn(__fsub_rn(-xxj, t), xxi), 0.0f);
            uint32_t u = __float_as_uint(pd);
            u ^= (u >> 31) ? 0xffffffffu : 0x80000000u;
            s_key[base + lane] = ((unsigned long long)u << 32) | (uint32_t)(~myid);
        }
    }
    __syncwarp();
    const size_t o = (size_t)grow * k;
    const int npairs = (total + 1) >> 1;
    for (int base = 0; base < total; base += 32) {
        const int s = base + lane;
        const unsigned long long mine = s < total ? s_key[s] : ~0ull;
        int rank = 0;
        const ulonglong2* kp = reinterpret_cast<const ulonglong2*>(s_key);
#pragma unroll 4
        for (int t = 0; t < npairs; ++t) {
            const ulonglong2 kk = kp[t];
            rank += (kk.x > mine) + (kk.y > mine);
        }
        if (s < total && rank < k) {
            const int id = (int)~(uint32_t)mine;
            if (idx_i64) reinterpret_cast<long long*>(idx_out)[o + rank] = id;
            else reinterpret_cast<int*>(idx_out)[o + rank] = id;
        }
    }
}

template <int CAP, int WARPS>
struct RefineTmaSmem {
    static constexpr int KEYS = 2 * CAP + 2;
    static constexpr size_t rows = (size_t)WARPS * 2 * 32 * 128;
    static constexpr size_t off_xi = rows;
    static constexpr size_t off_key = off_xi + (size_t)WARPS * 256;
    static constexpr size_t key_bytes = (KEYS * 8 + 15) / 16 * 16;
    static constexpr size_t off_id = off_key + (size_t)WARPS * key_bytes;
    static constexpr size_t off_bar = off_id + (size_t)WARPS * (2 * CAP + 4) * 4;
    static constexpr size_t total = off_bar + WARPS * 8;
    static_assert(total <= 227 * 1024, "refine shared memory budget");
};

__device__ __forceinline__ void tma_gather4_e(void* smem_dst, const CUtensorMap* tmap, uint64_t* bar, int col, const int4& r) {
    asm volatile(
        "{\n\t.reg .pred q;\n\t"
        "elect.sync _|q, 0xffffffff;\n\t"
        "@q cp.async.bulk.tensor.2d.shared::cluster.global.tile::gather4.mbarrier::complete_tx::bytes [%0], [%1, {%3, %4, %5, %6, %7}], [%2];\n\t}"
        ::"r"(smem_u32(smem_dst)), "l"(reinterpret_cast<uint64_t>(tmap)), "r"(smem_u32(bar)), "r"(col), "r"(r.x), "r"(r.y), "r"(r.z), "r"(r.w)
        : "memory");
}
__device__ __forceinline__ void bulk_load_e(void* smem_dst, const void* gsrc, uint32_t bytes, uint64_t* bar) {
    asm volatile(
        "{\n\t.reg .pred q;\n\t"
        "elect.sync _|q, 0xffffffff;\n\t"
        "@q cp.async.bulk.shared::cluster.global.mbarrier::complete_tx::bytes [%0], [%1], %2, [%3];\n\t}"
        ::"r"(smem_u32(smem_dst)), "l"(gsrc), "r"(bytes), "r"(smem_u32(bar)) : "memory");
}

template <int CAP, int WARPS>
__global__ void __launch_bounds__(WARPS * 32)
knn2_refine_tma_kernel(const __grid_constant__ CUtensorMap tmap_x, const float* __restrict__ x, const float* __restrict__ xxpad,
                       const int* __restrict__ cnt, const int* __restrict__ cand, int B, int N, int Npad, int k,
                       void* __restrict__ idx_out, int idx_i64, int* __restrict__ flags, int* __restrict__ list) {
    using S = RefineTmaSmem<CAP, WARPS>;
    constexpr int IPL = (CAP + 31) / 32;
    extern __shared__ __align__(1024) uint8_t rsm_t[];
    uint8_t* rsm = rsm_t;
    const int lane = threadIdx.x & 31, w = threadIdx.x >> 5;
    uint8_t* s_rows = rsm + (size_t)w * 2 * 32 * 128;
    const float4* s_xi = reinterpret_cast<const float4*>(rsm + S::off_xi + (size_t)w * 256);
    unsigned long long* s_key = reinterpret_cast<unsigned long long*>(rsm + S::off_key + (size_t)w * S::key_bytes);
    int* s_id = reinterpret_cast<int*>(rsm + S::off_id) + w * (2 * CAP + 4);
    uint64_t* bar = reinterpret_cast<uint64_t*>(rsm + S::off_bar) + w;
    if (lane == 0) {
        mbar_init(bar, 1);
        asm volatile("fence.mbarrier_init.release.cluster;" ::: "memory");
    }
    __syncwarp();
    const long long rows_total = (long long)B * N;
    const long long nw = (long long)gridDim.x * WARPS;
    uint32_t phase = 0;
    const int sw = lane & 7;
    int nc0 = 0, nc1 = 0, nl0[IPL], nl1[IPL];
    auto prefetch = [&](long long g) {
        if (g >= rows_total) return;
        nc0 = __ldg(cnt + g * 2); nc1 = __ldg(cnt + g * 2 + 1);
        const int* l0 = cand + (size_t)g * 2 * CAP;
#pragma unroll
        for (int i = 0; i < IPL; ++i) {
            const int s = lane + 32 * i;
            nl0[i] = s < CAP ? __ldg(l0 + s) : 0;
            nl1[i] = s < CAP ? __ldg(l0 + CAP + s) : 0;
        }
    };
    long long grow = (long long)blockIdx.x * WARPS + w;
    prefetch(grow);
    for (; grow < rows_total; grow += nw) {
        const int b = (int)(grow / N), qi = (int)(grow % N);
        const int c0 = nc0, c1 = nc1;
        const int total = c0 + c1;
        const bool bad = c0 > CAP || c1 > CAP || total < k;
        const int rbase = b * N;
        if (!bad) {
#pragma unroll
            for (int i = 0; i < IPL; ++i) {
                const int s = lane + 32 * i;
                if (s < c0) s_id[s] = rbase + nl0[i];
                if (s < c1) s_id[c0 + s] = rbase + nl1[i];
            }
            if (lane < 4) s_id[total + lane] = rbase + qi;
            if (lane < 2) s_key[total + lane] = 0ull;
        }
        __syncwarp();
        if (bad) {
            if (lane == 0) knn2_flag_tile(flags, list, b * ((N + 63) / 64) + qi / 64);
            prefetch(grow + nw);
            continue;
        }
        const float xxi = __ldg(xxpad + (size_t)b * Npad + qi);
        for (int base = 0; base < total; base += 32) {
            const int nc = min(32, total - base);
            const int n4 = (nc + 3) >> 2;
            mbar_expect_tx_e(bar, (uint32_t)n4 * 1024u + (base == 0 ? 256u : 0u));
            if (base == 0) bulk_load_e(const_cast<float4*>(s_xi), x + (size_t)grow * 64, 256u, bar);
            for (int g = 0; g < n4; ++g) {
                const int4 r = *reinterpret_cast<const int4*>(s_id + base + 4 * g);
                tma_gather4_e(s_rows + g * 512, &tmap_x, bar, 0, r);
                tma_gather4_e(s_rows + 4096 + g * 512, &tmap_x, bar, 32, r);
            }
            const int myrow = lane < nc ? s_id[base + lane] : rbase;
            const float xxj = __ldg(xxpad + (size_t)b * Npad + (myrow - rbase));
            if (base == 0) prefetch(grow + nw);
            mbar_wait(bar, phase);
            phase ^= 1u;
            float dot = 0.f;
#pragma unroll
            for (int ph = 0; ph < 2; ++ph) {
                const float4* rj = reinterpret_cast<const float4*>(s_rows + ph * 4096 + lane * 128);
#pragma unroll
                for (int g = 0; g < 8; ++g) {
                    const float4 u = s_xi[ph * 8 + g], v = rj[g ^ sw];
                    dot = __fmaf_rn(u.x, v.x, dot); dot = __fmaf_rn(u.y, v.y, dot);
                    dot = __fmaf_rn(u.z, v.z, dot); dot = __fmaf_rn(u.w, v.w, dot);
                }
            }
            if (lane < nc) {
                const float t = -2.0f * dot;
                const float pd = __fadd_rn(__fsub_rn(__fsub_rn(-xxj, t), xxi), 0.0f);
                uint32_t u = __float_as_uint(pd);
                u ^= (u >> 31) ? 0xffffffffu : 0x80000000u;
                s_key[base + lane] = ((unsigned long long)u << 32) | (uint32_t)(~(myrow - rbase));
            }
            __syncwarp();
        }
        const size_t o = (size_t)grow * k;
        const int npairs = (total + 1) >> 1;
        for (int base = 0; base < total; base += 32) {
            const int s = base + lane;
            const unsigned long long mine = s < total ? s_key[s] : ~0ull;
            int rank = 0;
            const ulonglong2* kp = reinterpret_cast<const ulonglong2*>(s_key);
#pragma unroll 4
            for (int t = 0; t < npairs; ++t) {
                const ulonglong2 kk = kp[t];
                rank += (kk.x > mine) + (kk.y > mine);
            }
            if (s < total && rank < k) {
                const int id = (int)~(uint32_t)mine;
                if (idx_i64) reinterpret_cast<long long*>(idx_out)[o + rank] = id;
                else reinterpret_cast<int*>(idx_out)[o + rank] = id;
            }
        }
        __syncwarp();
    }
}

static int g_refine_tma = [] { const char* e = getenv("LPD_KNN_REFINE"); return (e && atoi(e) == 0) ? 0 : 1; }();
static int g_refine_warps = [] { const char* e = getenv("LPD_KNN_REFINE_WARPS"); return e ? atoi(e) : 22; }();

template <int CAP, int WARPS>
static int knn2_refine_tma_launch(const float* x, const float* xxpad, const int* cnt, const int* cand, int B, int N, int Npad, int k,
                                  void* idx, int idx_i64, int* flags, int* list, cudaStream_t st) {
    CUtensorMap tx;
    int rc = make_tmap(&tx, x, (long long)B * N, 64, 64, 1);
    if (rc != LPD_OK) return rc;
    const size_t smem = RefineTmaSmem<CAP, WARPS>::total;
    static int sms = 0, per_sm = 0;
    if (per_sm == 0) {
        int dev = 0;
        LPD_CUDA_CHECK(allow_smem(knn2_refine_tma_kernel<CAP, WARPS>, smem));
        LPD_CUDA_CHECK(cudaGetDevice(&dev));
        LPD_CUDA_CHECK(cudaDeviceGetAttribute(&sms, cudaDevAttrMultiProcessorCount, dev));
        LPD_CUDA_CHECK(cudaOccupancyMaxActiveBlocksPerMultiprocessor(&per_sm, knn2_refine_tma_kernel<CAP, WARPS>, WARPS * 32, smem));
        if (per_sm < 1) per_sm = 1;
    }
    const long long want = ((long long)B * N + WARPS - 1) / WARPS;
    const long long blocks = want < (long long)sms * per_sm ? want : (long long)sms * per_sm;
    knn2_refine_tma_kernel<CAP, WARPS><<<(unsigned)blocks, WARPS * 32, smem, st>>>(tx, x, xxpad, cnt, cand, B, N, Npad, k, idx, idx_i64, flags, list);
    LPD_LAUNCH_CHECK();
    return LPD_OK;
}

template <int CAP>
static int knn2_refine_launch(const float* x, const float* xxpad, const int* cnt, const int* cand, int B, int N, int Npad, int k,
                              void* idx, int idx_i64, int* flags, int* list, cudaStream_t st) {
    if (g_refine_tma) {
        if constexpr (CAP > 64) {
            return knn2_refine_tma_launch<CAP, 16>(x, xxpad, cnt, cand, B, N, Npad, k, idx, idx_i64, flags, list, st);
        } else {
            if (g_refine_warps == 4) return knn2_refine_tma_launch<CAP, 4>(x, xxpad, cnt, cand, B, N, Npad, k, idx, idx_i64, flags, list, st);
            if (g_refine_warps == 11) return knn2_refine_tma_launch<CAP, 11>(x, xxpad, cnt, cand, B, N, Npad, k, idx, idx_i64, flags, list, st);
            return knn2_refine_tma_launch<CAP, 22>(x, xxpad, cnt, cand, B, N, Npad, k, idx, idx_i64, flags, list, st);
        }
    }
    const size_t smem = RefineSmem<CAP>::total;
    LPD_CUDA_CHECK(allow_smem(knn2_refine_kernel<CAP>, smem));
    const unsigned rblocks = (unsigned)(((long long)B * N + RF_WARPS - 1) / RF_WARPS);
    knn2_refine_kernel<CAP><<<rblocks, RF_WARPS * 32, smem, st>>>(x, xxpad, cnt, cand, B, N, Npad, k, idx, idx_i64, flags, list);
    LPD_LAUNCH_CHECK();
    return LPD_OK;
}

static int make_tmap_f16(CUtensorMap* m, const __half* base, long long rows, int box_rows) {
    EncodeTiledFn enc = get_encode();
    if (!enc) { snprintf(g_last_error, sizeof(g_last_error), "cuTensorMapEncodeTiled entry point not found"); return LPD_ECUDA; }
    cuuint64_t dims[2] = {64u, (cuuint64_t)rows};
    cuuint64_t strides[1] = {128u};
    cuuint32_t box[2] = {64u, (cuuint32_t)box_rows};
    cuuint32_t estr[2] = {1, 1};
    CUresult r = enc(m, CU_TENSOR_MAP_DATA_TYPE_FLOAT16, 2, const_cast<__half*>(base), dims, strides, box, estr,
                     CU_TENSOR_MAP_INTERLEAVE_NONE, CU_TENSOR_MAP_SWIZZLE_128B, CU_TENSOR_MAP_L2_PROMOTION_L2_256B,
                     CU_TENSOR_MAP_FLOAT_OOB_FILL_NONE);
    if (r != CUDA_SUCCESS) { snprintf(g_last_error, sizeof(g_last_error), "cuTensorMapEncodeTiled (fp16) failed: CUresult %d", (int)r); return LPD_ECUDA; }
    return LPD_OK;
}

static inline size_t align_up2(size_t v, size_t a) { return (v + a - 1) / a * a; }

static int g_cap_small = [] { const char* e = getenv("LPD_KNN_CAP"); return (e && atoi(e) == 40) ? 40 : 64; }();

struct Knn2Ws {
    size_t off_xx, off_nrm, off_sn, off_ext, off_r2, off_r2c, off_mu, off_sc, off_flags, off_list, off_xh, off_cnt, off_cand, total;
    int npad, cap;
    Knn2Ws(int B, int N, int k) {
        npad = (N + 255) / 256 * 256;
        cap = k > 24 ? 128 : (g_cap_small == 40 ? 40 : 64);
        size_t o = 0;
        off_xx = o; o = align_up2(o + (size_t)B * npad * 4, 256);
        off_nrm = o; o = align_up2(o + (size_t)B * npad * 4, 256);
        off_sn = o; o = align_up2(o + (size_t)B * npad * 4, 256);
        off_ext = o; o = align_up2(o + (size_t)B * npad * 32, 256);
        off_r2 = o; o += (size_t)B * 4;
        off_r2c = o; o = align_up2(o + (size_t)B * 4, 256);
        off_mu = o; o = align_up2(o + (size_t)B * K2_CSPLIT * 196 * 4, 256);
        off_sc = o; o = align_up2(o + (size_t)B * 2 * 4, 256);
        off_flags = o; o = align_up2(o + (size_t)B * ((N + 63) / 64) * 4, 256);
        off_list = o; o = align_up2(o + ((size_t)B * ((N + 63) / 64) + 1) * 4, 256);
        off_xh = o; o = align_up2(o + (size_t)B * N * 64 * 2, 256);
        off_cnt = o; o = align_up2(o + (size_t)B * N * 2 * 4, 256);
        off_cand = o; o = align_up2(o + (size_t)B * N * 2 * cap * 4, 256);
        total = o;
    }
};

size_t knn2_workspace_bytes(int B, int N, int k) { return Knn2Ws(B, N, k).total; }

template <int MT, int CAP, bool TIGHT, bool TS = false>
static int knn2_launch(const CUtensorMap& ta, const CUtensorMap& tb, const Knn2Params& P, cudaStream_t st) {
    const size_t smem = K2Smem<MT, TS>::total;
    LPD_CUDA_CHECK(allow_smem(knn2_tc_kernel<MT, CAP, TIGHT, TS>, smem));
    int dev = 0, sms = 0;
    LPD_CUDA_CHECK(cudaGetDevice(&dev));
    LPD_CUDA_CHECK(cudaDeviceGetAttribute(&sms, cudaDevAttrMultiProcessorCount, dev));
    const int items = P.B * P.qtiles;
    knn2_tc_kernel<MT, CAP, TIGHT, TS><<<items < sms ? items : sms, 256 * MT + 64, smem, st>>>(ta, tb, P);
    LPD_LAUNCH_CHECK();
    return LPD_OK;
}

int knn2_run(const float* x, int B, int N, int k, void* idx, int idx_i64, void* workspace, size_t workspace_bytes, int mt,
             cudaStream_t st) {
    const Knn2Ws W(B, N, k);
    if (workspace_bytes < W.total) return LPD_EWORKSPACE;
    uint8_t* ws = reinterpret_cast<uint8_t*>(workspace);
    float* xxpad = reinterpret_cast<float*>(ws + W.off_xx);
    float* nrmpad = reinterpret_cast<float*>(ws + W.off_nrm);
    float* snpad = reinterpret_cast<float*>(ws + W.off_sn);
    float* r2 = reinterpret_cast<float*>(ws + W.off_r2);
    float* r2c = reinterpret_cast<float*>(ws + W.off_r2c);
    float* mu = reinterpret_cast<float*>(ws + W.off_mu);
    float* sc = reinterpret_cast<float*>(ws + W.off_sc);
    int* flags = reinterpret_cast<int*>(ws + W.off_flags);
    int* list = reinterpret_cast<int*>(ws + W.off_list);
    __half* xh = reinterpret_cast<__half*>(ws + W.off_xh);
    LPD_CUDA_CHECK(cudaMemsetAsync(r2, 0, W.off_mu - W.off_r2, st));
    LPD_CUDA_CHECK(cudaMemsetAsync(flags, 0, W.off_list - W.off_flags + sizeof(int), st));
    knn2_center_kernel<<<dim3(K2_CSPLIT, B), 256, 0, st>>>(x, N, mu);
    LPD_LAUNCH_CHECK();
    static bool prep_smem_ok = false;
    if (!prep_smem_ok) { LPD_CUDA_CHECK(allow_smem(knn2_prep_kernel, K2_PREP_SMEM)); prep_smem_ok = true; }
    knn2_prep_kernel<<<dim3(ceil_div(W.npad, 256), B), 256, K2_PREP_SMEM, st>>>(x, mu, sc, N, W.npad, xh, reinterpret_cast<uint4*>(ws + W.off_ext), xxpad, nrmpad, snpad, r2, r2c);
    LPD_LAUNCH_CHECK();
    CUtensorMap ta, tb;
    int rc = make_tmap_f16(&ta, xh, (long long)B * N, 128);
    if (rc != LPD_OK) return rc;
    rc = make_tmap_f16(&tb, xh, (long long)B * N, K2_C);
    if (rc != LPD_OK) return rc;
    Knn2Params P;
    P.nrmpad = nrmpad; P.snpad = snpad; P.ext = reinterpret_cast<const uint4*>(ws + W.off_ext); P.xh = reinterpret_cast<const uint4*>(xh); P.xxpad = xxpad; P.r2 = r2; P.r2c = r2c; P.sc = sc;
    P.cnt = reinterpret_cast<int*>(ws + W.off_cnt);
    P.cand = reinterpret_cast<int*>(ws + W.off_cand);
    P.B = B; P.N = N; P.Npad = W.npad; P.k = k;
    P.qtiles = ceil_div(N, mt == 2 ? 256 : 128); P.ctiles = ceil_div(N, K2_C);
    if (mt == 3) {
        rc = (W.cap == 40) ? knn2_launch<1, 40, false, true>(ta, tb, P, st)
                           : (k <= 24 ? knn2_launch<1, 64, false, true>(ta, tb, P, st) : knn2_launch<1, 128, true, true>(ta, tb, P, st));
    } else if (W.cap == 40) rc = (mt == 2) ? knn2_launch<2, 40, false>(ta, tb, P, st) : knn2_launch<1, 40, false>(ta, tb, P, st);
    else if (k <= 24) rc = (mt == 2) ? knn2_launch<2, 64, false>(ta, tb, P, st) : knn2_launch<1, 64, false>(ta, tb, P, st);
    else             rc = (mt == 2) ? knn2_launch<2, 128, true>(ta, tb, P, st) : knn2_launch<1, 128, true>(ta, tb, P, st);
    if (rc != LPD_OK) return rc;
    rc = (W.cap == 40) ? knn2_refine_launch<40>(x, xxpad, P.cnt, P.cand, B, N, W.npad, k, idx, idx_i64, flags, list, st)
         : (W.cap == 64 ? knn2_refine_launch<64>(x, xxpad, P.cnt, P.cand, B, N, W.npad, k, idx, idx_i64, flags, list, st)
                        : knn2_refine_launch<128>(x, xxpad, P.cnt, P.cand, B, N, W.npad, k, idx, idx_i64, flags, list, st));
    if (rc != LPD_OK) return rc;
    return knn_simt64_list(x, B, N, k, idx, idx_i64, list, st);
}

size_t knn2_flags_offset(int B, int N, int k) { return Knn2Ws(B, N, k).off_flags; }
size_t knn2_cnt_offset(int B, int N, int k) { return Knn2Ws(B, N, k).off_cnt; }

}
}
```

### lpd-net-pytorch_b200/ops.py

```python
from __future__ import annotations

import torch

from . import _lib
from ._lib import (ACT_ADD, ACT_GATE, ACT_LEAKY, ACT_NONE, ACT_RELU, ACT_SIGMOID, A_KM, A_MK, B_KN, B_NK)

__all__ = ["bn_fold", "transpose", "knn", "knn_tc_variant", "pointwise_mlp2", "gemm", "colmax", "edge_gather_ext", "edgeconv_dg",
           "gemm_tf32", "linear", "set_precision", "get_precision", "netvlad_assign", "softmax64", "netvlad_finish", "splitk_reduce", "quadruplet_loss", "retrieval_topk", "retrieval_tc", "retrieval_search", "recall_count",
           "ACT_NONE", "ACT_RELU", "ACT_LEAKY", "ACT_SIGMOID", "ACT_GATE", "A_MK", "A_KM", "B_NK", "B_KN"]


def _stream() -> int:
    return torch.cuda.current_stream().cuda_stream


_weights_epoch = 0


def weights_epoch() -> int:
    return _weights_epoch


def bump_weights_epoch() -> None:
    global _weights_epoch
    _weights_epoch += 1


def dispatch_key() -> tuple:
    return (_precision, SPATIAL_ORDER, KNN_TENSOR_CORES, KNN_GRID, knn_tc_variant(-1) if _lib._lib is not None else -1)


_launches = 0
_profile = None


def reset_launch_count() -> None:
    global _launches
    _launches = 0


def launch_count() -> int:
    return _launches


def profile(enable: bool):
    global _profile
    rec, _profile = _profile, ([] if enable else None)
    return rec


def _call(label: str, nlaunch: int, fn, *args) -> None:
    global _launches
    if _profile is not None:
        s, e = torch.cuda.Event(enable_timing=True), torch.cuda.Event(enable_timing=True)
        s.record()
        rc = fn(*args)
        e.record()
        _profile.append((label, s, e))
    else:
        rc = fn(*args)
    _launches += nlaunch
    _lib.check(rc, label)


def _p(t):
    return None if t is None else t.data_ptr()


def _f32(t: torch.Tensor, name: str) -> torch.Tensor:
    if not t.is_cuda:
        raise _lib.LpdError(f"{name} must be a CUDA tensor: the lpd_b200 kernels have no CPU path")
    if t.dtype != torch.float32:
        raise _lib.LpdError(f"{name} must be float32, got {t.dtype}")
    if t.device.index != torch.cuda.current_device():
        raise _lib.LpdError(f"{name} lives on {t.device} but the current CUDA device is cuda:{torch.cuda.current_device()}; "
                            f"call torch.cuda.set_device (one process per GPU) or wrap the call in torch.cuda.device(...)")
    return t


def bn_fold(gamma, beta, mean, var, eps: float, bias=None):
    lib = _lib.load()
    _f32(mean, "running_mean")
    C = mean.numel()
    out = torch.empty(2, C, device=mean.device, dtype=torch.float32)
    _call("lpd_bn_fold", 1, lib.lpd_bn_fold, _p(gamma), _p(beta), _p(mean), _p(var), _p(bias), float(eps), C,
                               out[0].data_ptr(), out[1].data_ptr(), _stream())
    return out[0], out[1]


def transpose(x: torch.Tensor) -> torch.Tensor:
    lib = _lib.load()
    x = _f32(x, "x").contiguous()
    b, R, Cc = x.shape
    out = torch.empty(b, Cc, R, device=x.device, dtype=torch.float32)
    _call("lpd_transpose", 1, lib.lpd_transpose, x.data_ptr(), out.data_ptr(), b, R, Cc, _stream())
    return out


KNN_TENSOR_CORES = True
KNN_GRID = True


def knn_tc_variant(v: int = -1) -> int:
    return int(_lib.load().lpd_knn_tc_variant(int(v)))


def knn(x_pm: torch.Tensor, k: int, int64: bool = False, diag: dict | None = None) -> torch.Tensor:
    lib = _lib.load()
    x_pm = _f32(x_pm, "x").contiguous()
    B, N, Cc = x_pm.shape
    idx = torch.empty(B, N, k, device=x_pm.device, dtype=torch.int64 if int64 else torch.int32)
    if KNN_TENSOR_CORES and Cc == 64 and N >= 128 and x_pm.data_ptr() % 16 == 0:
        nbytes = lib.lpd_knn_workspace_bytes(B, N, Cc, k)
        ws = torch.empty((nbytes + 3) // 4, device=x_pm.device, dtype=torch.float32)
        _call(f"lpd_knn_tc[C={Cc},k={k}]", 5, lib.lpd_knn_tc, x_pm.data_ptr(), B, N, Cc, k, idx.data_ptr(), int(int64),
              ws.data_ptr(), ws.numel() * 4, _stream())
        if diag is not None:
            off = lib.lpd_knn_tc_flags_offset(B, N, Cc, k) // 4
            diag["flagged_tiles"] = int((ws.view(torch.int32)[off: off + B * ((N + 63) // 64)] != 0).sum().item())
            diag["tiles"] = B * ((N + 63) // 64)
    elif KNN_GRID and Cc == 3 and N >= 64 and _grid_of(x_pm) is not None:
        ws = _grid_of(x_pm)
        _call(f"lpd_knn_xyz[k={k}]", 2, lib.lpd_knn_xyz_ordered, B, N, k, idx.data_ptr(), int(int64), ws.data_ptr(), ws.numel() * 4, _stream())
    elif KNN_GRID and Cc == 3 and N >= 64:
        nbytes = lib.lpd_knn_xyz_workspace_bytes(B, N)
        ws = torch.empty((nbytes + 3) // 4, device=x_pm.device, dtype=torch.float32)
        _call(f"lpd_knn_xyz[k={k}]", 2, lib.lpd_knn_xyz, x_pm.data_ptr(), B, N, k, idx.data_ptr(), int(int64), ws.data_ptr(),
              ws.numel() * 4, _stream())
    else:
        _call(f"lpd_knn[C={Cc},k={k}]", 1, lib.lpd_knn, x_pm.data_ptr(), B, N, Cc, k, idx.data_ptr(), int(int64), _stream())
    return idx


SPATIAL_ORDER = True


_grid_cache = None


def _grid_of(x_pm: torch.Tensor):
    c = _grid_cache
    if (c is not None and x_pm.data_ptr() == c[0].data_ptr() and tuple(x_pm.shape) == tuple(c[0].shape) and c[0]._version == c[2]
            and x_pm.device == c[0].device):
        return c[1]
    return None


def cell_order(xyz: torch.Tensor, want_inv: bool = False):
    lib = _lib.load()
    xyz = _f32(xyz, "xyz").contiguous()
    B, N, _ = xyz.shape
    perm = torch.empty(B, N, device=xyz.device, dtype=torch.int32)
    inv = torch.empty(B, N, device=xyz.device, dtype=torch.int32) if want_inv else None
    out = torch.empty_like(xyz)
    nbytes = lib.lpd_knn_xyz_workspace_bytes(B, N)
    ws = torch.empty((nbytes + 3) // 4, device=xyz.device, dtype=torch.float32)
    _call("lpd_cell_order", 1, lib.lpd_cell_order_grid, xyz.data_ptr(), B, N, perm.data_ptr(), _p(inv), out.data_ptr(), ws.data_ptr(),
          ws.numel() * 4, _stream())
    global _grid_cache
    _grid_cache = (out, ws, out._version)
    return perm, inv, out


def gemm(A, B, *, a_layout=A_MK, b_layout=B_NK, M, N, K, lda=None, ldb=None, out=None, ldc=None,
         batch=1, strideA=0, strideB=0, strideC=0, scale=None, shift=None, act=ACT_NONE, slope=0.0, aux=None):
    lib = _lib.load()
    _f32(A, "A"), _f32(B, "B")
    if lda is None:
        lda = K if a_layout == A_MK else M
    if ldb is None:
        ldb = K if b_layout == B_NK else N
    if out is None:
        ldc = N
        out = torch.empty((batch, M, N) if batch > 1 else (M, N), device=A.device, dtype=torch.float32)
        if batch > 1:
            strideC = M * N
    elif ldc is None:
        ldc = out.stride(-2)
    _call(f"lpd_gemm[{M}x{N}x{K}x{batch}]", 1, lib.lpd_gemm, A.data_ptr(), a_layout, lda, strideA, B.data_ptr(), b_layout, ldb, strideB,
                            out.data_ptr(), ldc, strideC, M, N, K, batch, _p(scale), _p(shift), act, float(slope),
                            _p(aux), _stream())
    return out


_precision = "fp32"


def set_precision(mode: str) -> str:
    global _precision
    if mode not in ("fp32", "tf32", "f16"):
        raise ValueError("precision must be 'fp32', 'tf32' or 'f16'")
    prev, _precision = _precision, mode
    return prev


def get_precision() -> str:
    return _precision


def gemm_tf32(A, W, *, M, N, K, lda=None, ldw=None, out=None, ldc=None, scale=None, shift=None, act=ACT_NONE, slope=0.0, batch=1,
              accumulate=False):
    lib = _lib.load()
    _f32(A, "A"), _f32(W, "W")
    lda = K if lda is None else lda
    ldw = K if ldw is None else ldw
    if out is None:
        if accumulate:
            raise ValueError("gemm_tf32: accumulate needs an output buffer")
        out = torch.empty(batch * M, N, device=A.device, dtype=torch.float32)
        ldc = N
    elif ldc is None:
        ldc = out.stride(-2)
    label = f"lpd_gemm_tf32[{M}x{N}x{K}]" if batch == 1 else f"lpd_gemm_tf32[{M}x{N}x{K}x{batch}]"
    _call(label, 1, lib.lpd_gemm_tf32_ex, A.data_ptr(), lda, W.data_ptr(), ldw, out.data_ptr(), ldc,
          M, N, K, batch, int(bool(accumulate)), _p(scale), _p(shift), act, float(slope), _stream())
    return out


def gemm_tf32_tn(A, Bm, *, M, N, K, lda, ldb, batch=1, out=None):
    lib = _lib.load()
    _f32(A, "A"), _f32(Bm, "B")
    if out is None:
        out = torch.empty(batch, M, N, device=A.device, dtype=torch.float32)
    _call(f"lpd_gemm_tf32_tn[{M}x{N}x{K}x{batch}]", 1, lib.lpd_gemm_tf32_tn, A.data_ptr(), lda, Bm.data_ptr(), ldb, out.data_ptr(), N,
          M * N, M, N, K, batch, _stream())
    return out


def to_f16(x: torch.Tensor) -> torch.Tensor:
    lib = _lib.load()
    _f32(x, "x")
    rows, cols = x.shape
    y = torch.empty(rows, cols, device=x.device, dtype=torch.float16)
    _call("lpd_f32_to_f16", 1, lib.lpd_f32_to_f16, x.data_ptr(), x.stride(0), y.data_ptr(), cols, rows, cols, _stream())
    return y


def split3_tf32(x: torch.Tensor, role: int) -> torch.Tensor:
    lib = _lib.load()
    x = _f32(x, "x").contiguous()
    rows, cols = x.shape
    out = torch.empty(3 * rows, cols, device=x.device, dtype=torch.float32)
    _call("lpd_split3_tf32", 1, lib.lpd_split3_tf32, x.data_ptr(), x.numel(), out.data_ptr(), int(role), _stream())
    return out


def transpose_split3(v: torch.Tensor, Bp: int) -> torch.Tensor:
    lib = _lib.load()
    v = _f32(v, "v").contiguous()
    B, R = v.shape
    out = torch.empty(3 * R, Bp, device=v.device, dtype=torch.float32)
    _call("lpd_transpose_split3", 1, lib.lpd_transpose_split3, v.data_ptr(), B, R, Bp, out.data_ptr(), _stream())
    return out


def _f16(t: torch.Tensor, name: str) -> torch.Tensor:
    if not t.is_cuda or t.dtype != torch.float16:
        raise _lib.LpdError(f"{name} must be a CUDA float16 tensor, got {t.dtype} on {t.device}")
    if t.device.index != torch.cuda.current_device():
        raise _lib.LpdError(f"{name} lives on {t.device} but the current CUDA device is cuda:{torch.cuda.current_device()}")
    return t


def gemm_f16(A, W, *, M, N, K, lda=None, ldw=None, out=None, ldc=None, out_half=False, scale=None, shift=None, act=ACT_NONE, slope=0.0):
    lib = _lib.load()
    _f16(A, "A"), _f16(W, "W")
    lda = K if lda is None else lda
    ldw = K if ldw is None else ldw
    if out is None:
        out = torch.empty(M, N, device=A.device, dtype=torch.float16 if out_half else torch.float32)
        ldc = N
    else:
        out_half = out.dtype == torch.float16
        if ldc is None:
            ldc = out.stride(-2)
    _call(f"lpd_gemm_f16[{M}x{N}x{K}]", 1, lib.lpd_gemm_f16, A.data_ptr(), lda, W.data_ptr(), ldw, out.data_ptr(), ldc, int(out_half),
          M, N, K, _p(scale), _p(shift), act, float(slope), _stream())
    return out


def gemm_f16_tn(A, Bm, *, M, N, K, lda, ldb, batch=1, out=None):
    lib = _lib.load()
    _f16(A, "A"), _f16(Bm, "B")
    if out is None:
        out = torch.empty(batch, M, N, device=A.device, dtype=torch.float32)
    _call(f"lpd_gemm_f16_tn[{M}x{N}x{K}x{batch}]", 1, lib.lpd_gemm_f16_tn, A.data_ptr(), lda, Bm.data_ptr(), ldb, out.data_ptr(), N,
          M * N, M, N, K, batch, _stream())
    return out


def gemm_tf32_out16(A, W, *, M, N, K, lda=None, ldw=None, scale=None, shift=None, act=ACT_NONE, slope=0.0):
    lib = _lib.load()
    _f32(A, "A"), _f32(W, "W")
    out = torch.empty(M, N, device=A.device, dtype=torch.float16)
    _call(f"lpd_gemm_tf32[{M}x{N}x{K}]", 1, lib.lpd_gemm_tf32_out16, A.data_ptr(), K if lda is None else lda, W.data_ptr(),
          K if ldw is None else ldw, out.data_ptr(), N, M, N, K, _p(scale), _p(shift), act, float(slope), _stream())
    return out


def softmax64_f16(a, M):
    lib = _lib.load()
    a_h = torch.empty(M, 64, device=a.device, dtype=torch.float16)
    _call("lpd_softmax64", 1, lib.lpd_softmax64_f16, a.data_ptr(), M, a_h.data_ptr(), _stream())
    return a, a_h


def edge_gather_max_f16(p, ldp, q, ldq, idx, B, N, k, C, act, slope, out, ldo):
    lib = _lib.load()
    _f16(p, "p")
    _call(f"lpd_edge_gather_ext[C={C}]", 1, lib.lpd_edge_gather_max_f16, p.data_ptr(), ldp, _p(q), ldq, idx.data_ptr(), B, N, k, C,
          act, float(slope), out.data_ptr(), ldo, _stream())
    return out


def edgeconv_dg20_f16(p, ldp, q, ldq, idx, B, N, w2_h, s2, t2, act, slope, x1, ld1, x2, ld2):
    lib = _lib.load()
    _f16(p, "p"), _f16(w2_h, "w2")
    k = idx.shape[-1]
    if k not in (20, 32):
        raise _lib.LpdError(f"edgeconv_dg20_f16: k must be 20 or 32, got {k}")
    _call("lpd_edgeconv_dg_f16[128x128]", 1, lib.lpd_edgeconv_dg20_f16 if k == 20 else lib.lpd_edgeconv_dg32_f16, p.data_ptr(), ldp, q.data_ptr(), ldq, idx.data_ptr(), B, N,
          w2_h.data_ptr(), s2.data_ptr(), t2.data_ptr(), act, float(slope), _p(x1), ld1, x2.data_ptr(), ld2, _stream())
    return x1, x2


def _tn_ok(A, Bm, M, N, K, lda, ldb, batch):
    return (_precision != "fp32" and M >= 64 and N >= 64 and N % 4 == 0 and lda % 4 == 0 and ldb % 4 == 0 and K >= 256
            and (batch == 1 or K % 32 == 0) and A.data_ptr() % 16 == 0 and Bm.data_ptr() % 16 == 0)


def linear(A, W, *, M, N, K, lda=None, out=None, ldc=None, scale=None, shift=None, act=ACT_NONE, slope=0.0):
    lda_ = K if lda is None else lda
    if (_precision != "fp32" and K >= 32 and K % 4 == 0 and lda_ % 4 == 0 and N >= 64 and N % 4 == 0 and M >= 128
            and (ldc is None or ldc % 4 == 0) and A.data_ptr() % 16 == 0 and (out is None or out.data_ptr() % 16 == 0)):
        return gemm_tf32(A, W, M=M, N=N, K=K, lda=lda, out=out, ldc=ldc, scale=scale, shift=shift, act=act, slope=slope)
    return gemm(A, W, M=M, N=N, K=K, lda=lda, out=out, ldc=ldc, scale=scale, shift=shift, act=act, slope=slope)


def pointwise_mlp2(x, D, M, w1, s1, t1, w2, s2, t2, act=ACT_NONE, slope=0.0, ldx=None):
    lib = _lib.load()
    _f32(x, "x")
    out = torch.empty(M, 64, device=x.device, dtype=torch.float32)
    _call("lpd_pointwise_mlp2", 1, lib.lpd_pointwise_mlp2, x.data_ptr(), x.stride(-2) if ldx is None else ldx, D, M, w1.data_ptr(),
          s1.data_ptr(), t1.data_ptr(), w2.data_ptr(), s2.data_ptr(), t2.data_ptr(), act, float(slope), out.data_ptr(), 64, _stream())
    return out


def colmax(x: torch.Tensor, B: int, N: int, C: int, ldx: int | None = None) -> torch.Tensor:
    lib = _lib.load()
    _f32(x, "x")
    out = torch.empty(B, C, device=x.device, dtype=torch.float32)
    _call("lpd_colmax", 1, lib.lpd_colmax, x.data_ptr(), B, N, C, C if ldx is None else ldx, out.data_ptr(), _stream())
    return out


def edge_gather_ext(p, ldp, q, ldq, idx, B, N, k, C, scale, shift, act, slope, out, ldo):
    lib = _lib.load()
    _call(f"lpd_edge_gather_ext[C={C}]", 1, lib.lpd_edge_gather_ext, p.data_ptr(), ldp, _p(q), ldq, idx.data_ptr(), B, N, k, C, _p(scale), _p(shift),
                                       act, float(slope), out.data_ptr(), ldo, _stream())
    return out


def edgeconv_dg(p, ldp, q, ldq, idx, B, N, k, C1, C2, s1, t1, w2, s2, t2, act, slope, x1, ld1, x2, ld2):
    lib = _lib.load()
    tf32 = _precision != "fp32" and act != ACT_SIGMOID
    fn, label = (lib.lpd_edgeconv_dg_tf32, "lpd_edgeconv_dg_tf32") if tf32 else (lib.lpd_edgeconv_dg, "lpd_edgeconv_dg")
    if s1 is None and not (tf32 and k == 20 and C1 == 128 and C2 == 128):
        raise _lib.LpdError("edgeconv_dg: the pre-scaled form (s1 = t1 = None) exists for tf32 mode, k == 20, 128 channels only")
    _call(f"{label}[{C1}x{C2}]", 1, fn, p.data_ptr(), ldp, q.data_ptr(), ldq, idx.data_ptr(), B, N, k, C1, C2,
          _p(s1), _p(t1), w2.data_ptr(), s2.data_ptr(), t2.data_ptr(),
          act, float(slope), _p(x1), ld1, x2.data_ptr(), ld2, _stream())
    return x1, x2


def netvlad_assign(x, M, D, wc, scale, shift, K=64, out=None):
    lib = _lib.load()
    if out is None:
        out = torch.empty(M, K, device=x.device, dtype=torch.float32)
    _call("lpd_netvlad_assign", 2, lib.lpd_netvlad_assign, x.data_ptr(), M, D, wc.data_ptr(), _p(scale), _p(shift), K, out.data_ptr(),
                                      _stream())
    return out


def softmax64(a, M):
    lib = _lib.load()
    _call("lpd_softmax64", 1, lib.lpd_softmax64, a.data_ptr(), M, _stream())
    return a


def netvlad_finish(vlad, a, wc2, B, N, D, K=64):
    lib = _lib.load()
    ws = torch.empty(B * 8 * K, device=vlad.device, dtype=torch.float32)
    _call("lpd_netvlad_finish", 2, lib.lpd_netvlad_finish, vlad.data_ptr(), a.data_ptr(), wc2.data_ptr(), B, N, D, K, ws.data_ptr(),
                                      _stream())
    return vlad.view(B, D * K)


def gemm_softmax64(x, wct, *, M, K, scale=None, shift=None, want32=True, want16=False, want_parts=False):
    lib = _lib.load()
    f16 = x.dtype == torch.float16
    (_f16 if f16 else _f32)(x, "x"), (_f16 if f16 else _f32)(wct, "wct")
    a32 = torch.empty(M, 64, device=x.device, dtype=torch.float32) if want32 else None
    a16 = torch.empty(M, 64, device=x.device, dtype=torch.float16) if want16 else None
    apart = torch.empty((M + 31) // 32, 64, device=x.device, dtype=torch.float32) if want_parts else None
    _call(f"lpd_gemm_softmax64[{M}x64x{K}]", 1, lib.lpd_gemm_softmax64, x.data_ptr(), int(f16), K, wct.data_ptr(), K, M, K, _p(scale), _p(shift),
          _p(a32), _p(a16), _p(apart), _stream())
    return a32, a16, apart


def netvlad_finish_parts(vlad, apart, nparts, wc2, B, D, K=64):
    lib = _lib.load()
    _call("lpd_netvlad_finish", 1, lib.lpd_netvlad_finish_parts, vlad.data_ptr(), apart.data_ptr(), nparts, wc2.data_ptr(), B, D, K, _stream())
    return vlad.view(B, D * K)


def hidden_gate(part, splits, B, O, s2, t2, wg, sg, tg):
    lib = _lib.load()
    out = torch.empty(B, O, device=part.device, dtype=torch.float32)
    _call("lpd_hidden_gate", 1, lib.lpd_hidden_gate, part.data_ptr(), splits, B, O, _p(s2), _p(t2), wg.data_ptr(), _p(sg), _p(tg),
          out.data_ptr(), _stream())
    return out


def splitk_reduce(part, splits, M, N, scale=None, shift=None):
    lib = _lib.load()
    out = torch.empty(M, N, device=part.device, dtype=torch.float32)
    _call("lpd_splitk_reduce", 1, lib.lpd_splitk_reduce, part.data_ptr(), splits, M, N, _p(scale), _p(shift), out.data_ptr(), _stream())
    return out


def quadruplet_loss(q, pos, neg, other, m1, m2, use_min, lazy, ignore_zero_loss, need_grad=False, grad_out=None):
    lib = _lib.load()
    q, pos, neg = _f32(q, "q").contiguous(), _f32(pos, "pos").contiguous(), _f32(neg, "neg").contiguous()
    other = None if other is None else _f32(other, "other").contiguous()
    Bq, P, D = pos.shape
    Nn = neg.shape[1]
    flags = int(bool(use_min)) | (int(bool(lazy)) << 1) | (int(bool(ignore_zero_loss)) << 2)
    loss = torch.empty(1, device=q.device, dtype=torch.float32)
    grads = (None, None, None, None)
    if need_grad:
        grads = (torch.empty_like(q), torch.empty_like(pos), torch.empty_like(neg),
                 None if other is None else torch.empty_like(other))
    _call("lpd_quadruplet_loss", 1, lib.lpd_quadruplet_loss, q.data_ptr(), pos.data_ptr(), neg.data_ptr(), _p(other), Bq, P, Nn, D,
                                       float(m1), float(m2), flags, loss.data_ptr(), _p(grads[0]), _p(grads[1]),
                                       _p(grads[2]), _p(grads[3]), _p(grad_out), _stream())
    return (loss, grads) if need_grad else loss


def retrieval_topk(db: torch.Tensor, q: torch.Tensor, k: int, idx_offset: int = 0, want_dist: bool = True):
    lib = _lib.load()
    db, q = _f32(db, "db").contiguous(), _f32(q, "q").contiguous()
    Ndb, D = db.shape
    Nq = q.shape[0]
    idx = torch.empty(Nq, k, device=db.device, dtype=torch.int32)
    dist = torch.empty(Nq, k, device=db.device, dtype=torch.float64) if want_dist else None
    ws_bytes = lib.lpd_retrieval_workspace_bytes(Ndb, Nq, k)
    ws = torch.empty((ws_bytes + 7) // 8, device=db.device, dtype=torch.float64)
    _call("lpd_retrieval_topk", 2, lib.lpd_retrieval_topk, db.data_ptr(), Ndb, q.data_ptr(), Nq, D, k, idx_offset, idx.data_ptr(), _p(dist),
                                      ws.data_ptr(), ws.numel() * 8, _stream())
    return idx, dist


def topk_merge(part_dist: torch.Tensor, part_idx: torch.Tensor):
    lib = _lib.load()
    lists, Nq, k = part_idx.shape
    part_dist, part_idx = part_dist.contiguous(), part_idx.contiguous()
    idx = torch.empty(Nq, k, device=part_idx.device, dtype=torch.int32)
    dist = torch.empty(Nq, k, device=part_idx.device, dtype=torch.float64)
    _call("lpd_topk_merge", 1, lib.lpd_topk_merge, part_dist.data_ptr(), part_idx.data_ptr(), lists, Nq, k, idx.data_ptr(),
          dist.data_ptr(), _stream())
    return idx, dist


def retrieval_tc(db: torch.Tensor, q: torch.Tensor, k: int, seg_off: torch.Tensor, global_idx: bool = False, idx_offset: int = 0,
                 want_dist: bool = True):
    lib = _lib.load()
    db, q = _f32(db, "db").contiguous(), _f32(q, "q").contiguous()
    Ndb, D = db.shape
    Nq, S = q.shape[0], seg_off.numel() - 1
    idx = torch.empty(S, Nq, k, device=db.device, dtype=torch.int32)
    dist = torch.empty(S, Nq, k, device=db.device, dtype=torch.float64) if want_dist else None
    nbytes = lib.lpd_retrieval_tc_workspace_bytes(Ndb, Nq, D)
    ws = torch.empty(nbytes, device=db.device, dtype=torch.uint8)
    _call(f"lpd_retrieval_tc[{Nq}x{Ndb}x{D}]", 4, lib.lpd_retrieval_tc, db.data_ptr(), Ndb, q.data_ptr(), Nq, D, k, seg_off.data_ptr(), S,
          int(bool(global_idx)), int(idx_offset), idx.data_ptr(), _p(dist), ws.data_ptr(), nbytes, _stream())
    return idx, dist


RETRIEVAL_TC_MIN = 1 << 22
RETRIEVAL_SEG = 1024


def retrieval_search(db: torch.Tensor, q: torch.Tensor, k: int, idx_offset: int = 0, want_dist: bool = True):
    Ndb, D = db.shape
    Nq = q.shape[0]
    if Nq * Ndb < RETRIEVAL_TC_MIN or D % 4 or D > 1024 or k > Ndb:
        return retrieval_topk(db, q, k, idx_offset=idx_offset, want_dist=want_dist)
    seg = torch.arange(0, Ndb + RETRIEVAL_SEG, RETRIEVAL_SEG, device=db.device, dtype=torch.int32).clamp_(max=Ndb)
    idx, dist = retrieval_tc(db, q, k, seg, global_idx=True, idx_offset=idx_offset)
    if seg.numel() == 2:
        return idx[0], (dist[0] if want_dist else None)
    i, d = topk_merge(dist, idx)
    return i, (d if want_dist else None)


def recall_count(idx, q_run, R, truth_off, truth_idx, seg_thresh, seg_run=None, db=None, seg_off=None, q=None):
    lib = _lib.load()
    S, Nq, k = idx.shape
    dev = idx.device
    counters = torch.zeros(R * S * 27, device=dev, dtype=torch.int32)
    hist, n_eval, n_one = counters[: R * S * 25], counters[R * S * 25: R * S * 26], counters[R * S * 26:]
    sim = torch.empty(Nq, S, device=dev, dtype=torch.float32) if db is not None else None
    D = 0 if db is None else db.shape[1]
    _call("lpd_recall_count", 1, lib.lpd_recall_count, idx.data_ptr(), S, Nq, k, q_run.data_ptr(), R, _p(seg_run),
          truth_off.data_ptr(), truth_idx.data_ptr(), seg_thresh.data_ptr(), _p(db), _p(seg_off), _p(q), D, hist.data_ptr(),
          n_eval.data_ptr(), n_one.data_ptr(), _p(sim), _stream())
    return hist.view(R, S, 25), n_eval.view(R, S), n_one.view(R, S), sim


SM_COUNT = 148


def _nparts(rows: int, per: int = 64) -> int:
    return int(max(1, min(SM_COUNT * 8, (rows + per - 1) // per)))


def _partial(nparts: int, C: int, dev) -> torch.Tensor:
    return torch.empty(nparts * 2 * C, device=dev, dtype=torch.float64)


def bn_finalize(partial, nparts, count, C, gamma, beta, eps, momentum, running_mean, running_var):
    lib = _lib.load()
    bn = torch.empty(4, C, device=partial.device, dtype=torch.float32)
    _call("lpd_bn_finalize", 1, lib.lpd_bn_finalize, partial.data_ptr(), nparts, float(count), C, _p(gamma), _p(beta), float(eps),
          float(momentum), _p(running_mean), _p(running_var), bn.data_ptr(), _stream())
    if running_mean is not None or running_var is not None:
        bump_weights_epoch()
    return bn


def bn_stats(z, rows, C, ld):
    lib = _lib.load()
    nparts = _nparts(rows)
    part = _partial(nparts, C, z.device)
    _call(f"lpd_bn_stats[C={C}]", 1, lib.lpd_bn_stats, z.data_ptr(), rows, C, ld, part.data_ptr(), nparts, _stream())
    return part, nparts


def colsum_finalize(partial, nparts, n):
    lib = _lib.load()
    out = torch.empty(n, device=partial.device, dtype=torch.float32)
    _call("lpd_colsum_finalize", 1, lib.lpd_colsum_finalize, partial.data_ptr(), nparts, n, out.data_ptr(), _stream())
    return out


def affine_act(z, rows, C, ldz, scale, shift, act=ACT_NONE, slope=0.0, aux=None, ldaux=0, out=None, ldo=None):
    lib = _lib.load()
    if out is None:
        out = torch.empty(rows, C, device=z.device, dtype=torch.float32)
        ldo = C
    _call(f"lpd_affine_act[C={C}]", 1, lib.lpd_affine_act, z.data_ptr(), rows, C, ldz, _p(scale), _p(shift), act, float(slope),
          _p(aux), ldaux, out.data_ptr(), ldo, _stream())
    return out


def bn_bwd(dy, lddy, z, ldz, rows, C, bn, act, slope, count=None, aux=None, ldaux=0, dz=None, lddz=None):
    lib = _lib.load()
    nparts = _nparts(rows)
    part = _partial(nparts, C, z.device)
    _call(f"lpd_bn_bwd_reduce[C={C}]", 1, lib.lpd_bn_bwd_reduce, dy.data_ptr(), lddy, z.data_ptr(), ldz, rows, C, bn.data_ptr(),
          act, float(slope), _p(aux), ldaux, part.data_ptr(), nparts, _stream())
    S = colsum_finalize(part, nparts, 2 * C).view(2, C)
    if dz is None:
        dz = torch.empty(rows, C, device=z.device, dtype=torch.float32)
        lddz = C
    _call(f"lpd_bn_bwd_apply[C={C}]", 1, lib.lpd_bn_bwd_apply, dy.data_ptr(), lddy, z.data_ptr(), ldz, rows, C, bn.data_ptr(),
          S.data_ptr(), float(rows if count is None else count), act, float(slope), _p(aux), ldaux, dz.data_ptr(), lddz, _stream())
    return dz, S


def bn_bwd_sums(dy, lddy, z, ldz, rows, C, bn, act, slope):
    lib = _lib.load()
    nparts = _nparts(rows)
    part = _partial(nparts, C, z.device)
    _call(f"lpd_bn_bwd_reduce[C={C}]", 1, lib.lpd_bn_bwd_reduce, dy.data_ptr(), lddy, z.data_ptr(), ldz, rows, C, bn.data_ptr(),
          act, float(slope), None, 0, part.data_ptr(), nparts, _stream())
    return colsum_finalize(part, nparts, 2 * C).view(2, C)


def edge_sel_stats(p, ldp, q, ldq, idx, B, N, k, C, gamma):
    lib = _lib.load()
    M = B * N
    zsel = torch.empty(M, C, device=p.device, dtype=torch.float32)
    arg = torch.empty(M, C, device=p.device, dtype=torch.uint8)
    nparts = SM_COUNT * 8
    part = _partial(nparts, C, p.device)
    _call(f"lpd_edge_sel_stats[C={C}]", 1, lib.lpd_edge_sel_stats, p.data_ptr(), ldp, _p(q), ldq, idx.data_ptr(), B, N, k, C,
          _p(gamma), zsel.data_ptr(), C, arg.data_ptr(), part.data_ptr(), nparts, _stream())
    return zsel, arg, part, nparts


def edge_materialize(p, ldp, q, ldq, idx, B, N, k, C, scale, shift, act, slope):
    lib = _lib.load()
    y = torch.empty(B * N * k, C, device=p.device, dtype=torch.float32)
    _call(f"lpd_edge_materialize[C={C}]", 1, lib.lpd_edge_materialize, p.data_ptr(), ldp, _p(q), ldq, idx.data_ptr(), B, N, k, C,
          scale.data_ptr(), shift.data_ptr(), act, float(slope), y.data_ptr(), _stream())
    return y


def edge_sel_dense(z, M, k, C, gamma):
    lib = _lib.load()
    zsel = torch.empty(M, C, device=z.device, dtype=torch.float32)
    arg = torch.empty(M, C, device=z.device, dtype=torch.uint8)
    _call(f"lpd_edge_sel_dense[C={C}]", 1, lib.lpd_edge_sel_dense, z.data_ptr(), M, k, C, _p(gamma), zsel.data_ptr(), C,
          arg.data_ptr(), _stream())
    return zsel, arg


def edge_dense_bwd_apply(z, M, k, C, bn, S, count, act, slope, dx, lddx, zsel, arg):
    lib = _lib.load()
    _call(f"lpd_edge_dense_bwd_apply[C={C}]", 1, lib.lpd_edge_dense_bwd_apply, z.data_ptr(), M, k, C, bn.data_ptr(), S.data_ptr(),
          float(count), act, float(slope), dx.data_ptr(), lddx, zsel.data_ptr(), C, arg.data_ptr(), z.data_ptr(), _stream())
    return z


def edge_bwd(p, ldp, q, ldq, idx, B, N, k, C, bn, act, slope, dx, lddx, arg, dy, dp, lddp, dq, lddq, S=None):
    lib = _lib.load()
    count = B * N * k
    if S is None:
        nparts = SM_COUNT * 8
        part = _partial(nparts, C, p.device)
        _call(f"lpd_edge_bwd_reduce[C={C}]", 1, lib.lpd_edge_bwd_reduce, p.data_ptr(), ldp, _p(q), ldq, idx.data_ptr(), B, N, k, C,
              bn.data_ptr(), act, float(slope), _p(dx), lddx, _p(arg), _p(dy), part.data_ptr(), nparts, _stream())
        S = colsum_finalize(part, nparts, 2 * C).view(2, C)
    _call(f"lpd_edge_bwd_apply[C={C}]", 2, lib.lpd_edge_bwd_apply, p.data_ptr(), ldp, _p(q), ldq, idx.data_ptr(), B, N, k, C,
          bn.data_ptr(), act, float(slope), _p(dx), lddx, _p(arg), _p(dy), S.data_ptr(), float(count),
          dp.data_ptr(), lddp, _p(dq), lddq, _stream())
    return S


def edge_scatter_add(dy, idx, B, N, k, C, dp=None, lddp=None):
    lib = _lib.load()
    if dp is None:
        dp = torch.empty(B * N, C, device=dy.device, dtype=torch.float32)
        lddp = C
    _call(f"lpd_edge_scatter_add[C={C}]", 2, lib.lpd_edge_scatter_add, dy.data_ptr(), idx.data_ptr(), B, N, k, C, dp.data_ptr(), lddp, _stream())
    return dp


def act_bwd(dy, lddy, z, ldz, rows, C, act, slope, dz=None, lddz=None):
    lib = _lib.load()
    ident = torch.zeros(6, C, device=z.device, dtype=torch.float32)
    ident[0].fill_(1.0)
    ident[3].fill_(1.0)
    if dz is None:
        dz = torch.empty(rows, C, device=z.device, dtype=torch.float32)
        lddz = C
    _call(f"lpd_bn_bwd_apply[C={C}]", 1, lib.lpd_bn_bwd_apply, dy.data_ptr(), lddy, z.data_ptr(), ldz, rows, C, ident.data_ptr(),
          ident[4].data_ptr(), 1.0, act, float(slope), None, 0, dz.data_ptr(), lddz, _stream())
    return dz


def netvlad_finish_train(vlad, a, wc2, B, N, D, K=64):
    lib = _lib.load()
    dev = vlad.device
    asum = torch.empty(B, K, device=dev, dtype=torch.float32)
    n1 = torch.empty(B, K, device=dev, dtype=torch.float32)
    n2 = torch.empty(B, device=dev, dtype=torch.float32)
    _call("lpd_netvlad_finish_train", 1, lib.lpd_netvlad_finish_train, vlad.data_ptr(), a.data_ptr(), wc2.data_ptr(), B, N, D, K,
          asum.data_ptr(), n1.data_ptr(), n2.data_ptr(), _stream())
    return vlad.view(B, D * K), asum, n1, n2


def netvlad_finish_bwd(dv, v, wc2, asum, n1, n2, B, D, K=64):
    lib = _lib.load()
    dasum = torch.empty(B, K, device=dv.device, dtype=torch.float32)
    dwc2 = torch.empty(D, K, device=dv.device, dtype=torch.float32)
    _call("lpd_netvlad_finish_bwd", 2, lib.lpd_netvlad_finish_bwd, dv.data_ptr(), v.data_ptr(), wc2.data_ptr(), asum.data_ptr(),
          n1.data_ptr(), n2.data_ptr(), B, D, K, dasum.data_ptr(), dwc2.data_ptr(), _stream())
    return dv.view(B, D, K), dasum, dwc2


def softmax64_bwd(da, a, dasum, M, N):
    lib = _lib.load()
    _call("lpd_softmax64_bwd", 1, lib.lpd_softmax64_bwd, da.data_ptr(), a.data_ptr(), _p(dasum), M, N, _stream())
    return da


def colmax_arg(x, B, N, C, ldx=None):
    lib = _lib.load()
    out = torch.empty(B, C, device=x.device, dtype=torch.float32)
    arg = torch.empty(B, C, device=x.device, dtype=torch.int32)
    _call("lpd_colmax_arg", 1, lib.lpd_colmax_arg, x.data_ptr(), B, N, C, C if ldx is None else ldx, out.data_ptr(), arg.data_ptr(), _stream())
    return out, arg


def colmax_bwd(dout, arg, B, N, C, dx, lddx):
    lib = _lib.load()
    _call("lpd_colmax_bwd", 1, lib.lpd_colmax_bwd, dout.data_ptr(), arg.data_ptr(), B, N, C, dx.data_ptr(), lddx, _stream())
    return dx


def adam(w, g, m, v, lr, beta1, beta2, eps, weight_decay, step, grad_scale=1.0):
    lib = _lib.load()
    _call("lpd_adam", 1, lib.lpd_adam, w.data_ptr(), g.data_ptr(), m.data_ptr(), v.data_ptr(), w.numel(), float(lr), float(beta1),
          float(beta2), float(eps), float(weight_decay), int(step), float(grad_scale), _stream())
    bump_weights_epoch()


def axpy(y, ldy, x, ldx, rows, C, alpha=1.0):
    lib = _lib.load()
    _call("lpd_axpy", 1, lib.lpd_axpy, y.data_ptr(), ldy, x.data_ptr(), ldx, rows, C, float(alpha), _stream())
    return y


def wgrad(dz, lddz, a, lda, rows, Nout, Kin, out=None):
    bn = 256 if _precision != "fp32" else 128
    tiles = ((Nout + 127) // 128) * ((Kin + bn - 1) // bn)
    want = max(1, min(512, (2 * SM_COUNT + tiles - 1) // tiles, rows // 256 if rows >= 256 else 1))
    splits = 1
    while splits * 2 <= want and rows % (splits * 2) == 0:
        splits *= 2
    per = rows // splits
    part = torch.empty(splits, Nout, Kin, device=dz.device, dtype=torch.float32)
    if _tn_ok(dz, a, Nout, Kin, per, lddz, lda, splits):
        gemm_tf32_tn(dz, a, M=Nout, N=Kin, K=per, lda=lddz, ldb=lda, batch=splits, out=part)
    else:
        gemm(dz, a, a_layout=A_KM, b_layout=B_KN, M=Nout, N=Kin, K=per, lda=lddz, ldb=lda, out=part, ldc=Kin,
             batch=splits, strideA=per * lddz, strideB=per * lda, strideC=Nout * Kin)
    if splits == 1 and out is None:
        return part[0]
    res = splitk_reduce(part, splits, Nout, Kin)
    if out is not None:
        axpy(out, Kin, res, Kin, Nout, Kin, 1.0)
        return out
    return res
```

Baseline: 29350.

## Skip pruned column tiles in kNN pass two and prefetch next item's tiles

The tensor-core kNN kernel now has scan warps publish per-warp masks of the column tiles still needed after pass one. The TMA producer and MMA warps read the OR of those masks and load and multiply only those tiles in pass two, where before they recomputed every tile. The producer also overlaps item boundaries by loading the next item's A tile and its first few B stages during the current item's pass two. This adds an extra mbarrier handshake, a per-item atomic counter and more complex phase bookkeeping, so any miscount of stages across the three warp roles could deadlock.

```diff
diff --git a/include/lpd_b200.h b/include/lpd_b200.h
--- a/include/lpd_b200.h
+++ b/include/lpd_b200.h
@@ -49,6 +49,8 @@
                void* workspace, size_t workspace_bytes, void* stream);
 int lpd_knn_tc_variant(int v);
 size_t lpd_knn_tc_flags_offset(int B, int N, int C, int k);
+size_t lpd_knn_tc_cnt_offset(int B, int N, int C, int k);
+size_t lpd_knn_tc_pass2_offset(int B, int N, int C, int k);
 
 size_t lpd_knn_xyz_workspace_bytes(int B, int N);
 int lpd_knn_xyz(const float* x, int B, int N, int k, void* idx, int idx_i64, void* workspace, size_t workspace_bytes,
diff --git a/lpd-net-pytorch_b200/_lib.py b/lpd-net-pytorch_b200/_lib.py
--- a/lpd-net-pytorch_b200/_lib.py
+++ b/lpd-net-pytorch_b200/_lib.py
@@ -27,6 +27,8 @@
     "lpd_knn_tc": (_i, [_vp, _i, _i, _i, _i, _vp, _i, _vp, _sz, _vp]),
     "lpd_knn_tc_variant": (_i, [_i]),
     "lpd_knn_tc_flags_offset": (_sz, [_i, _i, _i, _i]),
+    "lpd_knn_tc_cnt_offset": (_sz, [_i, _i, _i, _i]),
+    "lpd_knn_tc_pass2_offset": (_sz, [_i, _i, _i, _i]),
     "lpd_knn_xyz_workspace_bytes": (_sz, [_i, _i]),
     "lpd_knn_xyz": (_i, [_vp, _i, _i, _i, _vp, _i, _vp, _sz, _vp]),
     "lpd_cell_order": (_i, [_vp, _i, _i, _vp, _vp, _vp, _vp, _sz, _vp]),
diff --git a/lpd-net-pytorch_b200/csrc/knn_tc.cu b/lpd-net-pytorch_b200/csrc/knn_tc.cu
--- a/lpd-net-pytorch_b200/csrc/knn_tc.cu
+++ b/lpd-net-pytorch_b200/csrc/knn_tc.cu
@@ -381,6 +381,8 @@
 namespace lpd { namespace tc {
 size_t knn2_workspace_bytes(int B, int N, int k);
 size_t knn2_flags_offset(int B, int N, int k);
+size_t knn2_cnt_offset(int B, int N, int k);
+size_t knn2_pass2_offset(int B, int N, int k);
 int knn2_run(const float* x, int B, int N, int k, void* idx, int idx_i64, void* workspace, size_t workspace_bytes, int mt,
              cudaStream_t st);
 static int g_knn_variant = 1;
@@ -401,6 +403,16 @@
 extern "C" size_t lpd_knn_tc_flags_offset(int B, int N, int C, int k) {
     if (B < 1 || N < 1 || C != 64 || k < 1 || k > 32) return 0;
     return lpd::tc::g_knn_variant == 0 ? lpd::tc::KnnWs(B, N, k).off_flags : lpd::tc::knn2_flags_offset(B, N, k);
+}
+
+extern "C" size_t lpd_knn_tc_cnt_offset(int B, int N, int C, int k) {
+    if (B < 1 || N < 1 || C != 64 || k < 1 || k > 32 || lpd::tc::g_knn_variant == 0) return 0;
+    return lpd::tc::knn2_cnt_offset(B, N, k);
+}
+
+extern "C" size_t lpd_knn_tc_pass2_offset(int B, int N, int C, int k) {
+    if (B < 1 || N < 1 || C != 64 || k < 1 || k > 32 || lpd::tc::g_knn_variant == 0) return 0;
+    return lpd::tc::knn2_pass2_offset(B, N, k);
 }
 
 extern "C" int lpd_knn_tc(const float* x, int B, int N, int C, int k, void* idx, int idx_i64,
diff --git a/lpd-net-pytorch_b200/csrc/knn_tc2.cu b/lpd-net-pytorch_b200/csrc/knn_tc2.cu
--- a/lpd-net-pytorch_b200/csrc/knn_tc2.cu
+++ b/lpd-net-pytorch_b200/csrc/knn_tc2.cu
@@ -14,6 +14,7 @@
 constexpr int K2_TCOLS = 512;
 constexpr int K2_XSLOTS = 12;
 constexpr int K2_TBL = 128;
+constexpr int K2_PRE = 4;
 
 struct Knn2Params {
     const float* nrmpad;
@@ -26,8 +27,10 @@
     const float* sc;
     int* cnt;
     int* cand;
+    unsigned long long* p2stages;
     int B, N, Npad, k;
     int qtiles, ctiles;
+    int compact;
 };
 
 __device__ __forceinline__ void tc_mma_f16(uint32_t tmem_d, uint64_t desc_a, uint64_t desc_b, uint32_t idesc, uint32_t accumulate) {
@@ -337,6 +340,25 @@
     return r;
 }
 
+__device__ __forceinline__ void k2_item_tiles(const uint32_t* msk, int nwarps, int lane, unsigned long long& lo,
+                                              unsigned long long& hi) {
+    uint32_t w[4];
+#pragma unroll
+    for (int i = 0; i < 4; ++i) w[i] = __reduce_or_sync(kFull, lane < nwarps ? msk[lane * 4 + i] : 0u);
+    lo = ((unsigned long long)w[1] << 32) | w[0];
+    hi = ((unsigned long long)w[3] << 32) | w[2];
+}
+__device__ __forceinline__ int k2_pop_tile(unsigned long long& lo, unsigned long long& hi) {
+    if (lo) {
+        const int t = __ffsll((long long)lo) - 1;
+        lo &= lo - 1;
+        return t;
+    }
+    const int t = 63 + __ffsll((long long)hi);
+    hi &= hi - 1;
+    return t;
+}
+
 template <int MT, bool TS = false>
 struct K2Smem {
     static constexpr int SCAN_THREADS = 256 * MT;
@@ -352,8 +374,9 @@
     static constexpr size_t off_xs = off_ax + 128 * 32;
     static constexpr size_t off_ex = off_xs + K2_XSLOTS * K2_C * 4;
     static constexpr size_t off_tbl = off_ex + (size_t)32 * EXS * 4;
-    static constexpr size_t off_bar = (off_tbl + (size_t)8 * MT * K2_TBL * 4 + 7) / 8 * 8;
-    static constexpr size_t total = off_bar + (4 + 2 * K2_BSTAGES + 2 * TSTAGES) * 8 + 16;
+    static constexpr size_t off_msk = off_tbl + (size_t)8 * MT * K2_TBL * 4;
+    static constexpr size_t off_bar = (off_msk + (size_t)2 * 8 * MT * 4 * 4 + 7) / 8 * 8;
+    static constexpr size_t total = off_bar + (6 + 2 * K2_BSTAGES + 2 * TSTAGES) * 8 + 16;
     static_assert(total <= 227 * 1024, "knn2 shared memory budget");
 };
 
@@ -375,9 +398,11 @@
     float* xs = reinterpret_cast<float*>(smem + S::off_xs);
     float* ex = reinterpret_cast<float*>(smem + S::off_ex);
     int* tbl = reinterpret_cast<int*>(smem + S::off_tbl);
+    uint32_t* msk = reinterpret_cast<uint32_t*>(smem + S::off_msk);
     uint64_t* afull = reinterpret_cast<uint64_t*>(smem + S::off_bar);
     uint64_t* aempty = afull + 2;
-    uint64_t* bfull = aempty + 2;
+    uint64_t* mfull = aempty + 2;
+    uint64_t* bfull = mfull + 2;
     uint64_t* bempty = bfull + K2_BSTAGES;
     uint64_t* tfull = bempty + K2_BSTAGES;
     uint64_t* tempty = tfull + K2_TSTAGES;
@@ -385,8 +410,8 @@
 
     const int warp = threadIdx.x >> 5, lane = threadIdx.x & 31;
     const int items = P.B * P.qtiles;
-    const int nstages = 2 * P.ctiles;
     const int full_blocks = P.N >> 6;
+    const int pre = P.ctiles < K2_PRE ? P.ctiles : K2_PRE;
 
     if (threadIdx.x < 128) {
         const int r = threadIdx.x;
@@ -400,7 +425,9 @@
         if (lane == 0) {
             asm volatile("prefetch.tensormap [%0];" ::"l"(reinterpret_cast<uint64_t>(&tmap_a)) : "memory");
             asm volatile("prefetch.tensormap [%0];" ::"l"(reinterpret_cast<uint64_t>(&tmap_b)) : "memory");
-            for (int s = 0; s < 2; ++s) { mbar_init(&afull[s], TS ? SCAN_WARPS : 1); mbar_init(&aempty[s], 1); }
+            for (int s = 0; s < 2; ++s) {
+                mbar_init(&afull[s], TS ? SCAN_WARPS : 1); mbar_init(&aempty[s], 1); mbar_init(&mfull[s], SCAN_WARPS);
+            }
             for (int s = 0; s < K2_BSTAGES; ++s) { mbar_init(&bfull[s], 1); mbar_init(&bempty[s], 1); }
             for (int s = 0; s < K2_TSTAGES; ++s) { mbar_init(&tfull[s], 1); mbar_init(&tempty[s], SCAN_WARPS); }
             asm volatile("fence.mbarrier_init.release.cluster;" ::: "memory");
@@ -417,30 +444,45 @@
     if (warp == SCAN_WARPS) {
         {
             const uint32_t leader = lane == 0;
-            uint32_t tcount = 0, icount = 0;
+            uint32_t s = 0, ph = 0, xsl = 0, icount = 0;
+            auto load_a = [&](int it, uint32_t n) {
+                if (TS) return;
+                const int b = it / P.qtiles, q0 = (it % P.qtiles) * (128 * MT);
+                const uint32_t ab = n & 1;
+                mbar_wait_sleep(&aempty[ab], ((n >> 1) & 1) ^ 1);
+                mbar_expect_tx_p(&afull[ab], S::A_BYTES, leader);
+#pragma unroll
+                for (int mt = 0; mt < MT; ++mt)
+                    tma_load_2d_p(a_s + ab * S::A_BYTES + mt * S::A_TILE, &tmap_a, &afull[ab], 0, b * P.N + q0 + mt * 128, leader);
+            };
+            auto load_stage = [&](int it, int ct) {
+                const int b = it / P.qtiles;
+                mbar_wait_sleep(&bempty[s], ph ^ 1);
+                mbar_expect_tx_p(&bfull[s], S::B_BYTES + S::BX_BYTES + (TIGHT ? K2_C * 4 : 0), leader);
+                tma_load_2d_p(b_s + s * S::B_BYTES, &tmap_b, &bfull[s], 0, b * P.N + ct * K2_C, leader);
+                bulk_load_p(bx_s + s * S::BX_BYTES, P.ext + ((size_t)b * (P.Npad >> 6) + 2 * ct) * 128, S::BX_BYTES, &bfull[s], leader);
+                if (TIGHT) bulk_load_p(xs + xsl * K2_C, P.snpad + (size_t)b * P.Npad + ct * K2_C, K2_C * 4, &bfull[s], leader);
+                if (++s == K2_BSTAGES) { s = 0; ph ^= 1; }
+                xsl = (xsl + 1) % K2_XSLOTS;
+            };
+            if (blockIdx.x < items) load_a(blockIdx.x, 0);
             for (int item = blockIdx.x; item < items; item += gridDim.x, ++icount) {
-                const int b = item / P.qtiles, q0 = (item % P.qtiles) * (128 * MT);
-                const uint32_t ab = icount & 1, aph = (icount >> 1) & 1;
-                if (!TS) {
-                    mbar_wait_sleep(&aempty[ab], aph ^ 1);
-                    mbar_expect_tx_p(&afull[ab], S::A_BYTES, leader);
-#pragma unroll
-                    for (int mt = 0; mt < MT; ++mt)
-                        tma_load_2d_p(a_s + ab * S::A_BYTES + mt * S::A_TILE, &tmap_a, &afull[ab], 0, b * P.N + q0 + mt * 128, leader);
-                }
-                const uint4* extb = P.ext + (size_t)b * (P.Npad >> 6) * 128;
-                const float* snb = P.snpad + (size_t)b * P.Npad;
-                uint32_t s = tcount % K2_BSTAGES, ph = (tcount / K2_BSTAGES) & 1, xsl = tcount % K2_XSLOTS;
-                for (int cs = 0; cs < nstages; ++cs, ++tcount) {
-                    const int ct = cs >= P.ctiles ? cs - P.ctiles : cs;
-                    mbar_wait_sleep(&bempty[s], ph ^ 1);
-                    mbar_expect_tx_p(&bfull[s], S::B_BYTES + S::BX_BYTES + (TIGHT ? K2_C * 4 : 0), leader);
-                    tma_load_2d_p(b_s + s * S::B_BYTES, &tmap_b, &bfull[s], 0, b * P.N + ct * K2_C, leader);
-                    bulk_load_p(bx_s + s * S::BX_BYTES, extb + (size_t)ct * 256, S::BX_BYTES, &bfull[s], leader);
-                    if (TIGHT) bulk_load_p(xs + xsl * K2_C, snb + ct * K2_C, K2_C * 4, &bfull[s], leader);
-                    if (++s == K2_BSTAGES) { s = 0; ph ^= 1; }
-                    xsl = (xsl + 1) % K2_XSLOTS;
-                }
+                const int next = item + gridDim.x;
+                for (int ct = icount ? pre : 0; ct < P.ctiles; ++ct) load_stage(item, ct);
+                if (next < items) {
+                    load_a(next, icount + 1);
+                    for (int ct = 0; ct < pre; ++ct) load_stage(next, ct);
+                }
+                int n2 = P.ctiles;
+                unsigned long long lo = 0, hi = 0;
+                if (P.compact) {
+                    const uint32_t ab = icount & 1;
+                    mbar_wait(&mfull[ab], (icount >> 1) & 1);
+                    k2_item_tiles(msk + ab * SCAN_WARPS * 4, SCAN_WARPS, lane, lo, hi);
+                    n2 = __popcll(lo) + __popcll(hi);
+                }
+                for (int i = 0; i < n2; ++i) load_stage(item, P.compact ? k2_pop_tile(lo, hi) : i);
+                if (lane == 0) atomicAdd(P.p2stages, (unsigned long long)n2);
             }
         }
     } else if (warp == SCAN_WARPS + 1) {
@@ -448,44 +490,58 @@
             constexpr uint32_t idesc = make_idesc_f16(128, K2_C);
             const uint32_t leader = lane == 0;
             const uint64_t dax = make_smem_desc_ext(smem_u32(ax_s));
-            uint32_t tcount = 0, icount = 0;
-            for (int item = blockIdx.x; item < items; item += gridDim.x, ++icount) {
-                const uint32_t ab = icount & 1, aph = (icount >> 1) & 1;
-                mbar_wait_sleep(&afull[ab], aph);
+            uint32_t s = 0, ph = 0, ts = 0, tph = 0, icount = 0;
+            auto wait_a = [&](uint32_t n) {
+                mbar_wait_sleep(&afull[n & 1], (n >> 1) & 1);
                 if (TS) tc_fence_after();
-                const uint64_t da0 = make_smem_desc(smem_u32(a_s + ab * S::A_BYTES));
-                const uint32_t ta0 = tmem_base + ACOL + ab * 64;
-                uint32_t s = tcount % K2_BSTAGES, ph = (tcount / K2_BSTAGES) & 1;
-                uint32_t ts = tcount % K2_TSTAGES, tph = (tcount / K2_TSTAGES) & 1;
-                for (int cs = 0; cs < nstages; ++cs, ++tcount) {
-                    mbar_wait(&tempty[ts], tph ^ 1);
-                    mbar_wait(&bfull[s], ph);
-                    tc_fence_after();
-                    const uint64_t db = make_smem_desc(smem_u32(b_s + s * S::B_BYTES));
-                    const uint64_t dbx = make_smem_desc_ext(smem_u32(bx_s + s * S::BX_BYTES));
-                    if (TS) {
-                        const uint32_t d = tmem_base + ts * TCOLS;
-#pragma unroll
-                        for (int ks = 0; ks < 4; ++ks) tc_mma_f16_ts(d, ta0 + ks * 8, db + (uint64_t)(ks * 2), idesc, ks ? 1u : 0u);
-                        tc_mma_f16_ts(d, ta0 + 32, dbx, idesc, 1u);
-                    } else {
-#pragma unroll
-                        for (int ks = 0; ks < 5; ++ks) {
-#pragma unroll
-                            for (int mt = 0; mt < MT; ++mt) {
-                                const uint64_t da = da0 + (uint64_t)(mt * (S::A_TILE >> 4));
-                                const uint32_t d = tmem_base + ts * TCOLS + mt * K2_C;
-                                if (ks < 4) tc_mma_f16_p(d, da + (uint64_t)(ks * 2), db + (uint64_t)(ks * 2), idesc, ks ? 1u : 0u, leader);
-                                else tc_mma_f16_p(d, dax, dbx, idesc, 1u, leader);
-                            }
+            };
+            auto mma_stage = [&](uint32_t n) {
+                const uint32_t ab = n & 1;
+                mbar_wait(&tempty[ts], tph ^ 1);
+                mbar_wait(&bfull[s], ph);
+                tc_fence_after();
+                const uint64_t db = make_smem_desc(smem_u32(b_s + s * S::B_BYTES));
+                const uint64_t dbx = make_smem_desc_ext(smem_u32(bx_s + s * S::BX_BYTES));
+                if (TS) {
+                    const uint32_t ta0 = tmem_base + ACOL + ab * 64;
+                    const uint32_t d = tmem_base + ts * TCOLS;
+#pragma unroll
+                    for (int ks = 0; ks < 4; ++ks) tc_mma_f16_ts(d, ta0 + ks * 8, db + (uint64_t)(ks * 2), idesc, ks ? 1u : 0u);
+                    tc_mma_f16_ts(d, ta0 + 32, dbx, idesc, 1u);
+                } else {
+                    const uint64_t da0 = make_smem_desc(smem_u32(a_s + ab * S::A_BYTES));
+#pragma unroll
+                    for (int ks = 0; ks < 5; ++ks) {
+#pragma unroll
+                        for (int mt = 0; mt < MT; ++mt) {
+                            const uint64_t da = da0 + (uint64_t)(mt * (S::A_TILE >> 4));
+                            const uint32_t d = tmem_base + ts * TCOLS + mt * K2_C;
+                            if (ks < 4) tc_mma_f16_p(d, da + (uint64_t)(ks * 2), db + (uint64_t)(ks * 2), idesc, ks ? 1u : 0u, leader);
+                            else tc_mma_f16_p(d, dax, dbx, idesc, 1u, leader);
                         }
                     }
-                    tc_commit_p(&bempty[s], leader);
-                    tc_commit_p(&tfull[ts], leader);
-                    if (++s == K2_BSTAGES) { s = 0; ph ^= 1; }
-                    if (++ts == K2_TSTAGES) { ts = 0; tph ^= 1; }
-                }
-                tc_commit_p(&aempty[ab], leader);
+                }
+                tc_commit_p(&bempty[s], leader);
+                tc_commit_p(&tfull[ts], leader);
+                if (++s == K2_BSTAGES) { s = 0; ph ^= 1; }
+                if (++ts == K2_TSTAGES) { ts = 0; tph ^= 1; }
+            };
+            if (blockIdx.x < items) wait_a(0);
+            for (int item = blockIdx.x; item < items; item += gridDim.x, ++icount) {
+                for (int ct = icount ? pre : 0; ct < P.ctiles; ++ct) mma_stage(icount);
+                if (item + (int)gridDim.x < items) {
+                    wait_a(icount + 1);
+                    for (int ct = 0; ct < pre; ++ct) mma_stage(icount + 1);
+                }
+                int n2 = P.ctiles;
+                if (P.compact) {
+                    unsigned long long lo, hi;
+                    mbar_wait(&mfull[icount & 1], (icount >> 1) & 1);
+                    k2_item_tiles(msk + (icount & 1) * SCAN_WARPS * 4, SCAN_WARPS, lane, lo, hi);
+                    n2 = __popcll(lo) + __popcll(hi);
+                }
+                for (int i = 0; i < n2; ++i) mma_stage(icount);
+                tc_commit_p(&aempty[icount & 1], leader);
             }
         }
     } else {
@@ -523,64 +579,78 @@
             __syncwarp();
             if (lane == 0) mbar_arrive(&afull[buf]);
         };
-        if (TS && blockIdx.x < items) { load_a(blockIdx.x); store_a(0); }
-        for (int item = blockIdx.x; item < items; item += gridDim.x, ++icount) {
-            const int b = item / P.qtiles, q0 = (item % P.qtiles) * (128 * MT);
-            const bool have_next = TS && item + (int)gridDim.x < items;
-            if (have_next) load_a(item + gridDim.x);
-            const int srow = q0 + mt * 128 + quad * 32 + lane;
-            int row = srow;
+        struct Row { int b, row; bool live; float inv_cb, ni, cni, gself, ub_extra; };
+        auto row_of = [&](int it) {
+            Row R;
+            R.b = it / P.qtiles;
+            const int srow = (it % P.qtiles) * (128 * MT) + mt * 128 + quad * 32 + lane;
+            R.row = srow;
             if ((srow >> 6) < full_blocks) {
                 int a, bb;
                 block_perm(srow >> 6, a, bb);
-                row = (srow & ~63) | ((((srow & 63) - bb) * inv_mod64(a)) & 63);
-            }
-            const bool live = srow < P.N;
-            const float inv_cb = 1.f / __ldg(P.sc + 2 * b + 1);
-            float ni = 0.f, cni = 0.f, gself = 0.f;
-            if (live) {
-                const float ni2 = __ldg(P.nrmpad + (size_t)b * P.Npad + srow);
-                ni = sqrtf(ni2); cni = 2.5e-3f * ni * inv_cb;
-                gself = ni2 * inv_cb;
-            }
-            const bool use_tbl = P.ctiles <= K2_TBL;
-            int* wtbl = tbl + warp * K2_TBL;
-            const float ub_extra = TIGHT ? cni * sqrtf(__ldg(P.r2c + b)) : 0.f;
-            float m[32];
-#pragma unroll
-            for (int j = 0; j < 32; ++j) m[j] = -INFINITY;
-            for (int cs = 0; cs < P.ctiles; ++cs, ++tcount) {
-                const uint32_t ts = tcount % K2_TSTAGES, tph = (tcount / K2_TSTAGES) & 1;
-                mbar_wait(&tfull[ts], tph);
-                tc_fence_after();
-                uint32_t r0[32], r1[32];
-                tc_ld32x2(tmem_base + tm_lane + ts * TCOLS, r0, r1);
-                tc_fence_before();
-                __syncwarp();
-                if (lane == 0) mbar_arrive(&tempty[ts]);
-                float tm = -INFINITY;
-                if (TIGHT) {
-                    const float* xsj = xs + (tcount % K2_XSLOTS) * K2_C + half * 32;
-#pragma unroll
-                    for (int j = 0; j < 32; j += 4) {
-                        const float4 s0 = *reinterpret_cast<const float4*>(xsj + j), s1 = *reinterpret_cast<const float4*>(xsj + 64 + j);
-                        m[j + 0] = fmax3(m[j + 0], fmaf(-cni, s0.x, __uint_as_float(r0[j + 0])), fmaf(-cni, s1.x, __uint_as_float(r1[j + 0])));
-                        m[j + 1] = fmax3(m[j + 1], fmaf(-cni, s0.y, __uint_as_float(r0[j + 1])), fmaf(-cni, s1.y, __uint_as_float(r1[j + 1])));
-                        m[j + 2] = fmax3(m[j + 2], fmaf(-cni, s0.z, __uint_as_float(r0[j + 2])), fmaf(-cni, s1.z, __uint_as_float(r1[j + 2])));
-                        m[j + 3] = fmax3(m[j + 3], fmaf(-cni, s0.w, __uint_as_float(r0[j + 3])), fmaf(-cni, s1.w, __uint_as_float(r1[j + 3])));
-                    }
-                } else {
-#pragma unroll
-                    for (int j = 0; j < 32; ++j) m[j] = fmax3(m[j], __uint_as_float(r0[j]), __uint_as_float(r1[j]));
-                }
-                if (use_tbl) {
-#pragma unroll
-                    for (int j = 0; j < 32; ++j) tm = fmax3(tm, __uint_as_float(r0[j]), __uint_as_float(r1[j]));
-                    const float D = live ? gself - (tm + ub_extra) : INFINITY;
-                    const int dk = __reduce_min_sync(kFull, fkey(D));
-                    if (lane == 0) wtbl[cs] = dk;
-                }
-            }
+                R.row = (srow & ~63) | ((((srow & 63) - bb) * inv_mod64(a)) & 63);
+            }
+            R.live = srow < P.N;
+            R.inv_cb = 1.f / __ldg(P.sc + 2 * R.b + 1);
+            R.ni = 0.f; R.cni = 0.f; R.gself = 0.f;
+            if (R.live) {
+                const float ni2 = __ldg(P.nrmpad + (size_t)R.b * P.Npad + srow);
+                R.ni = sqrtf(ni2); R.cni = 2.5e-3f * R.ni * R.inv_cb;
+                R.gself = ni2 * R.inv_cb;
+            }
+            R.ub_extra = TIGHT ? R.cni * sqrtf(__ldg(P.r2c + R.b)) : 0.f;
+            return R;
+        };
+        const bool use_tbl = P.ctiles <= K2_TBL;
+        int* wtbl = tbl + warp * K2_TBL;
+        float m[32];
+        auto pass1_stage = [&](const Row& R, int cs) {
+            const uint32_t ts = tcount % K2_TSTAGES, tph = (tcount / K2_TSTAGES) & 1;
+            mbar_wait(&tfull[ts], tph);
+            tc_fence_after();
+            uint32_t r0[32], r1[32];
+            tc_ld32x2(tmem_base + tm_lane + ts * TCOLS, r0, r1);
+            tc_fence_before();
+            __syncwarp();
+            if (lane == 0) mbar_arrive(&tempty[ts]);
+            float tm = -INFINITY;
+            if (TIGHT) {
+                const float* xsj = xs + (tcount % K2_XSLOTS) * K2_C + half * 32;
+#pragma unroll
+                for (int j = 0; j < 32; j += 4) {
+                    const float4 s0 = *reinterpret_cast<const float4*>(xsj + j), s1 = *reinterpret_cast<const float4*>(xsj + 64 + j);
+                    m[j + 0] = fmax3(m[j + 0], fmaf(-R.cni, s0.x, __uint_as_float(r0[j + 0])), fmaf(-R.cni, s1.x, __uint_as_float(r1[j + 0])));
+                    m[j + 1] = fmax3(m[j + 1], fmaf(-R.cni, s0.y, __uint_as_float(r0[j + 1])), fmaf(-R.cni, s1.y, __uint_as_float(r1[j + 1])));
+                    m[j + 2] = fmax3(m[j + 2], fmaf(-R.cni, s0.z, __uint_as_float(r0[j + 2])), fmaf(-R.cni, s1.z, __uint_as_float(r1[j + 2])));
+                    m[j + 3] = fmax3(m[j + 3], fmaf(-R.cni, s0.w, __uint_as_float(r0[j + 3])), fmaf(-R.cni, s1.w, __uint_as_float(r1[j + 3])));
+                }
+            } else {
+#pragma unroll
+                for (int j = 0; j < 32; ++j) m[j] = fmax3(m[j], __uint_as_float(r0[j]), __uint_as_float(r1[j]));
+            }
+            if (use_tbl) {
+#pragma unroll
+                for (int j = 0; j < 32; ++j) tm = fmax3(tm, __uint_as_float(r0[j]), __uint_as_float(r1[j]));
+                const float D = R.live ? R.gself - (tm + R.ub_extra) : INFINITY;
+                const int dk = __reduce_min_sync(kFull, fkey(D));
+                if (lane == 0) wtbl[cs] = dk;
+            }
+            ++tcount;
+        };
+        Row R;
+        if (blockIdx.x < items) R = row_of(blockIdx.x);
+#pragma unroll
+        for (int j = 0; j < 32; ++j) m[j] = -INFINITY;
+        if (TS && blockIdx.x < items) { load_a(blockIdx.x); store_a(0); }
+        for (int item = blockIdx.x; item < items; item += gridDim.x, ++icount) {
+            const int b = R.b, row = R.row;
+            const bool live = R.live;
+            const float cni = R.cni;
+            const int next = item + gridDim.x;
+            const bool have_next = next < items;
+            if (TS && have_next) load_a(next);
+            for (int cs = icount ? pre : 0; cs < P.ctiles; ++cs) pass1_stage(R, cs);
+            if (TS && have_next) store_a(icount + 1);
             bitonic_sort32_desc(m);
 #pragma unroll
             for (int j = 0; j < 32; ++j) ex[j * S::EXS + own] = m[j];
@@ -597,19 +667,46 @@
                 const float xxi = __ldg(P.xxpad + (size_t)b * P.Npad + row);
                 const float r2 = __ldg(P.r2 + b), r2c = __ldg(P.r2c + b), sigma = __ldg(P.sc + 2 * b);
                 const float rc = sqrtf(r2c);
-                float eps = (1.9e-6f / sigma) * (ni + rc) + 7.62939453125e-6f * (xxi + r2) + 3.814697265625e-6f * r2c;
-                if (!TIGHT) eps += 2.5e-3f * ni * rc;
-                thr = fmaxf(tau0 - 2.f * eps * inv_cb, -1.0e9f);
-                if (!(eps * inv_cb < INFINITY)) thr = __int_as_float(0x7fc00000);
-            }
-            if (have_next) store_a(icount + 1);
-            const int dthr = __reduce_max_sync(kFull, fkey(live ? gself - thr : -INFINITY));
+                float eps = (1.9e-6f / sigma) * (R.ni + rc) + 7.62939453125e-6f * (xxi + r2) + 3.814697265625e-6f * r2c;
+                if (!TIGHT) eps += 2.5e-3f * R.ni * rc;
+                thr = fmaxf(tau0 - 2.f * eps * R.inv_cb, -1.0e9f);
+                if (!(eps * R.inv_cb < INFINITY)) thr = __int_as_float(0x7fc00000);
+            }
+            const int dthr = __reduce_max_sync(kFull, fkey(live ? R.gself - thr : -INFINITY));
+            uint32_t need[4];
+#pragma unroll
+            for (int i = 0; i < 4; ++i) {
+                const int ct = 32 * i + lane;
+                need[i] = __ballot_sync(kFull, use_tbl && ct < P.ctiles && !(wtbl[ct] > dthr));
+            }
+            const unsigned long long need_lo = ((unsigned long long)need[1] << 32) | need[0];
+            const unsigned long long need_hi = ((unsigned long long)need[3] << 32) | need[2];
+            int n2 = P.ctiles;
+            unsigned long long lo = 0, hi = 0;
+            if (P.compact) {
+                const uint32_t ab = icount & 1;
+                if (lane == 0) {
+#pragma unroll
+                    for (int i = 0; i < 4; ++i) msk[(ab * SCAN_WARPS + warp) * 4 + i] = need[i];
+                    mbar_arrive(&mfull[ab]);
+                }
+                mbar_wait(&mfull[ab], (icount >> 1) & 1);
+                k2_item_tiles(msk + ab * SCAN_WARPS * 4, SCAN_WARPS, lane, lo, hi);
+                n2 = __popcll(lo) + __popcll(hi);
+            }
+            if (have_next) {
+                R = row_of(next);
+#pragma unroll
+                for (int j = 0; j < 32; ++j) m[j] = -INFINITY;
+                for (int cs = 0; cs < pre; ++cs) pass1_stage(R, cs);
+            }
             int cnt = 0;
             int* mine = P.cand + (((size_t)b * P.N + (live ? row : 0)) * 2 + half) * CAP;
-            for (int cs = 0; cs < P.ctiles; ++cs, ++tcount) {
+            for (int i = 0; i < n2; ++i, ++tcount) {
+                const int cs = P.compact ? k2_pop_tile(lo, hi) : i;
                 const uint32_t ts = tcount % K2_TSTAGES, tph = (tcount / K2_TSTAGES) & 1;
                 mbar_wait(&tfull[ts], tph);
-                if (use_tbl && wtbl[cs] > dthr) {
+                if (use_tbl && !(((cs < 64 ? need_lo >> cs : need_hi >> (cs - 64)) & 1ull))) {
                     __syncwarp();
                     if (lane == 0) mbar_arrive(&tempty[ts]);
                     continue;
@@ -981,9 +1078,11 @@
 static inline size_t align_up2(size_t v, size_t a) { return (v + a - 1) / a * a; }
 
 static int g_cap_small = [] { const char* e = getenv("LPD_KNN_CAP"); return (e && atoi(e) == 40) ? 40 : 64; }();
+static int g_pass2_skip = [] { const char* e = getenv("LPD_KNN_PASS2_SKIP"); return (e && atoi(e) == 0) ? 0 : 1; }();
 
 struct Knn2Ws {
-    size_t off_xx, off_nrm, off_sn, off_ext, off_r2, off_r2c, off_mu, off_sc, off_flags, off_list, off_xh, off_cnt, off_cand, total;
+    size_t off_xx, off_nrm, off_sn, off_ext, off_r2, off_r2c, off_mu, off_sc, off_p2, off_flags, off_list, off_xh, off_cnt, off_cand,
+           total;
     int npad, cap;
     Knn2Ws(int B, int N, int k) {
         npad = (N + 255) / 256 * 256;
@@ -997,6 +1096,7 @@
         off_r2c = o; o = align_up2(o + (size_t)B * 4, 256);
         off_mu = o; o = align_up2(o + (size_t)B * K2_CSPLIT * 196 * 4, 256);
         off_sc = o; o = align_up2(o + (size_t)B * 2 * 4, 256);
+        off_p2 = o; o = align_up2(o + 8, 256);
         off_flags = o; o = align_up2(o + (size_t)B * ((N + 63) / 64) * 4, 256);
         off_list = o; o = align_up2(o + ((size_t)B * ((N + 63) / 64) + 1) * 4, 256);
         off_xh = o; o = align_up2(o + (size_t)B * N * 64 * 2, 256);
@@ -1037,7 +1137,7 @@
     int* list = reinterpret_cast<int*>(ws + W.off_list);
     __half* xh = reinterpret_cast<__half*>(ws + W.off_xh);
     LPD_CUDA_CHECK(cudaMemsetAsync(r2, 0, W.off_mu - W.off_r2, st));
-    LPD_CUDA_CHECK(cudaMemsetAsync(flags, 0, W.off_list - W.off_flags + sizeof(int), st));
+    LPD_CUDA_CHECK(cudaMemsetAsync(ws + W.off_p2, 0, W.off_list - W.off_p2 + sizeof(int), st));
     knn2_center_kernel<<<dim3(K2_CSPLIT, B), 256, 0, st>>>(x, N, mu);
     LPD_LAUNCH_CHECK();
     static bool prep_smem_ok = false;
@@ -1053,8 +1153,10 @@
     P.nrmpad = nrmpad; P.snpad = snpad; P.ext = reinterpret_cast<const uint4*>(ws + W.off_ext); P.xh = reinterpret_cast<const uint4*>(xh); P.xxpad = xxpad; P.r2 = r2; P.r2c = r2c; P.sc = sc;
     P.cnt = reinterpret_cast<int*>(ws + W.off_cnt);
     P.cand = reinterpret_cast<int*>(ws + W.off_cand);
+    P.p2stages = reinterpret_cast<unsigned long long*>(ws + W.off_p2);
     P.B = B; P.N = N; P.Npad = W.npad; P.k = k;
     P.qtiles = ceil_div(N, mt == 2 ? 256 : 128); P.ctiles = ceil_div(N, K2_C);
+    P.compact = g_pass2_skip && P.ctiles <= K2_TBL;
     if (mt == 3) {
         rc = (W.cap == 40) ? knn2_launch<1, 40, false, true>(ta, tb, P, st)
                            : (k <= 24 ? knn2_launch<1, 64, false, true>(ta, tb, P, st) : knn2_launch<1, 128, true, true>(ta, tb, P, st));
@@ -1071,6 +1173,7 @@
 
 size_t knn2_flags_offset(int B, int N, int k) { return Knn2Ws(B, N, k).off_flags; }
 size_t knn2_cnt_offset(int B, int N, int k) { return Knn2Ws(B, N, k).off_cnt; }
-
-}
-}
+size_t knn2_pass2_offset(int B, int N, int k) { return Knn2Ws(B, N, k).off_p2; }
+
+}
+}
diff --git a/lpd-net-pytorch_b200/ops.py b/lpd-net-pytorch_b200/ops.py
--- a/lpd-net-pytorch_b200/ops.py
+++ b/lpd-net-pytorch_b200/ops.py
@@ -119,6 +119,11 @@
             off = lib.lpd_knn_tc_flags_offset(B, N, Cc, k) // 4
             diag["flagged_tiles"] = int((ws.view(torch.int32)[off: off + B * ((N + 63) // 64)] != 0).sum().item())
             diag["tiles"] = B * ((N + 63) // 64)
+            off = lib.lpd_knn_tc_pass2_offset(B, N, Cc, k)
+            if off:
+                diag["pass2_stages"] = int(ws.view(torch.int64)[off // 8].item())
+                off = lib.lpd_knn_tc_cnt_offset(B, N, Cc, k) // 4
+                diag["cand_counts"] = ws.view(torch.int32)[off: off + B * N * 2].view(B, N, 2).cpu()
     elif KNN_GRID and Cc == 3 and N >= 64 and _grid_of(x_pm) is not None:
         ws = _grid_of(x_pm)
         _call(f"lpd_knn_xyz[k={k}]", 2, lib.lpd_knn_xyz_ordered, B, N, k, idx.data_ptr(), int(int64), ws.data_ptr(), ws.numel() * 4, _stream())
```

New measurement: 29810 (median of 6 runs). 1.6% higher.
